# jby1993/SelfReconCode

Hardware: AMD Instinct MI355X
Metric: train.py-equivalent iterations/sec (540x540, 2048 rays/frame x 3 frames per GPU; coarse stage at Adam lr 0.0001) (higher is better)
Workload: dtype f32

## Files before the change

### include/selfrecon_hip.h

```cpp
#ifndef SELFRECON_HIP_H_
#define SELFRECON_HIP_H_
#include <stdint.h>

#ifdef __cplusplus
extern "C" {
#endif

#define SR_OK 0
#define SR_EINVAL (-1)
#define SR_ELAUNCH (-2)
#define SR_ENOSPC (-3)

int sr_abi_version(void);
const char* sr_build_arch(void);
const char* sr_build_digest(void);

int sr_minv3x3_fwd_f32(const float* ms, float* invs, uint8_t* checks, int64_t n, void* stream);
int sr_minv3x3_fwd_f64(const double* ms, double* invs, uint8_t* checks, int64_t n, void* stream);
int sr_minv3x3_bwd_f32(const float* grads, const float* invs, float* outs, int64_t n, void* stream);
int sr_minv3x3_bwd_f64(const double* grads, const double* invs, double* outs, int64_t n, void* stream);

typedef struct {
  int64_t size[5];
  int64_t stride[5];
} sr_tensor5;

int sr_gridsample3d_fwd_f32(const float* input, sr_tensor5 in_d, const float* grid, sr_tensor5 grid_d,
                            float* output, sr_tensor5 out_d, void* stream);
int sr_gridsample3d_fwd_f64(const double* input, sr_tensor5 in_d, const double* grid, sr_tensor5 grid_d,
                            double* output, sr_tensor5 out_d, void* stream);
int sr_gridsample3d_bwd_f32(const float* input, sr_tensor5 in_d, const float* grid, sr_tensor5 grid_d,
                            const float* grad_output, sr_tensor5 gout_d,
                            float* grad_input , sr_tensor5 gin_d, float* grad_grid, void* stream);
int sr_gridsample3d_bwd_f64(const double* input, sr_tensor5 in_d, const double* grid, sr_tensor5 grid_d,
                            const double* grad_output, sr_tensor5 gout_d,
                            double* grad_input , sr_tensor5 gin_d, double* grad_grid, void* stream);
int sr_gridsample3d_fwd_f16(const void* input, sr_tensor5 in_d, const void* grid, sr_tensor5 grid_d, void* output, sr_tensor5 out_d,
                            void* stream);
int sr_gridsample3d_bwd_f16(const void* input, sr_tensor5 in_d, const void* grid, sr_tensor5 grid_d, const void* grad_output,
                            sr_tensor5 gout_d, void* grad_input , sr_tensor5 gin_d, void* grad_grid, void* stream);
int sr_gridsample3d_dbwd_f16(const void* gO_input , sr_tensor5 goi_d, const void* gO_grid, sr_tensor5 gog_d,
                             const void* input, sr_tensor5 in_d, const void* grid, sr_tensor5 grid_d, const void* grad_output,
                             sr_tensor5 gout_d, void* grad_input , sr_tensor5 gin_d, void* grad_grid,
                             void* grad_grad_output, void* stream);
int sr_gridsample3d_dbwd_f32(const float* gO_input , sr_tensor5 goi_d, const float* gO_grid, sr_tensor5 gog_d,
                             const float* input, sr_tensor5 in_d, const float* grid, sr_tensor5 grid_d,
                             const float* grad_output, sr_tensor5 gout_d,
                             float* grad_input , sr_tensor5 gin_d, float* grad_grid, float* grad_grad_output,
                             void* stream);
int sr_gridsample3d_dbwd_f64(const double* gO_input , sr_tensor5 goi_d, const double* gO_grid, sr_tensor5 gog_d,
                             const double* input, sr_tensor5 in_d, const double* grid, sr_tensor5 grid_d,
                             const double* grad_output, sr_tensor5 gout_d,
                             double* grad_input , sr_tensor5 gin_d, double* grad_grid, double* grad_grad_output,
                             void* stream);


#define SR_ACT_NONE 0
#define SR_ACT_SOFTPLUS100 1
#define SR_ACT_RELU 2
#define SR_EPI_FWD 0
#define SR_EPI_BWD 1
typedef struct {
  const float* A; int64_t lda;
  const float* B; int64_t ldb;
  float* C; int64_t ldc;
  int32_t M, N, K;
  const float* bias;
  int32_t group, act, mode;
  float out_scale;
  const float* aux; int64_t ldaux;
  int32_t naux_fwd;
  int32_t nact_bwd;
  float aux_scale;
} sr_gemm_args;
int sr_mlp_gemm_nt(const sr_gemm_args* host_args, void* stream);
int sr_mlp_gemm_nt_tile(int32_t M, int32_t ncols, int32_t* bm_out, int32_t* bn_out);

#define SR_CHAIN_MAX_LAYERS 10
typedef struct {
  int32_t nlayers;
  int32_t nprob[SR_CHAIN_MAX_LAYERS];
  sr_gemm_args g[SR_CHAIN_MAX_LAYERS][2];
  const int32_t* m_dev; int32_t m_mul;
  int32_t m_cap;
} sr_chain_args;
int sr_mlp_chain(const sr_chain_args* host_args, void* stream);

typedef struct {
  const float* Z; int64_t ldz;
  const float* A; int64_t lda;
  float* dW; int64_t lddw;
  float* partial;
  int32_t R, N, K, splits, accumulate;
  float* db; float* db_partial; int32_t group;
} sr_gemm_tn_args;
int64_t sr_mlp_gemm_tn_workspace_floats(int32_t R, int32_t N, int64_t lddw, int32_t* host_splits_out);
int sr_mlp_gemm_tn(const sr_gemm_tn_args* host_args, void* stream);
#define SR_TN_GROUP_MAX 12
typedef struct {
  int32_t n;
  sr_gemm_tn_args p[SR_TN_GROUP_MAX];
} sr_gemm_tn_group_args;
int sr_mlp_gemm_tn_group(const sr_gemm_tn_group_args* host_args, void* stream);

int sr_pe_embed(const float* x, int64_t P, int32_t L, const float* band_weights, const float* extra, int64_t ldextra,
                int32_t E, const int64_t* extra_index , int32_t group, float* out, int64_t ldo, void* stream);
int sr_pe_embed_bwd(const float* x, int64_t P, int32_t L, const float* band_weights, int32_t group, const float* gA0,
                    int64_t ldg, float* xbar, void* stream);

typedef struct {
  const float* p; const float* tp; int64_t P;
  const float* A; const float* trans; int32_t nframes;
  const int64_t* batch_inds; int64_t points_per_frame;
  const float* vol; int32_t D, H, W;
  float bmin[3], bmax[3];
  float* y;
  float* jac;
} sr_lbs_args;
int sr_lbs_fwd(const sr_lbs_args* host_args, void* stream);
int64_t sr_lbs_bwd_workspace_floats(int64_t P, int32_t nframes);
int sr_lbs_bwd(const sr_lbs_args* host_args, const float* ybar, float* pbar, float* Abar, float* transbar, float* partials, void* stream);
int sr_lbs_jac_bwd(const sr_lbs_args* host_args, const float* ybar, const float* Jbar, float* pbar, float* Abar, float* transbar, float* partials,
                   void* stream);

int sr_lbs_chain_fwd(const float* poses, int32_t B, const float* host_Js, const int32_t* host_parents, const float* host_init_pose,
                     float* G, float* A, void* stream);
int sr_lbs_chain_bwd(const float* poses, int32_t B, const float* host_Js, const int32_t* host_parents, const float* host_init_pose,
                     const float* Abar, const float* Gbar, float* posebar, void* stream);

typedef struct {
  int64_t M; int32_t group;
  const float* sdf4; int64_t ld_sdf;
  const float* off4; int64_t ld_off;
  const float* y; const float* jlbs;
  const float* rays; const float* cam;
  const float* p; float* p_out;
  uint8_t* converged;
  float dthreshold, athreshold, w1, w2;
} sr_newton_args;
int sr_newton_update(const sr_newton_args* host_args, void* stream);

typedef struct {
  int64_t M;
  const float* sdf; int64_t ld_sdf;
  const float* y; const float* jlbs;
  const float* rays; const float* cam;
  uint8_t* converged;
  float* t_out; int64_t ld_t; float* s_out;
  const float* grad_f; const float* grad_off;
  const float* p; float* p_out;
  float dthreshold, athreshold, w1, w2;
} sr_newton2_args;
int sr_newton_prepare(const sr_newton2_args* host_args, void* stream);
int sr_newton_apply(const sr_newton2_args* host_args, void* stream);

typedef struct {
  int32_t P, times;
  const float* p0; const float* rays; const int64_t* batch_inds;
  const float* cam;
  int32_t L_sdf; const float* w_sdf; int32_t L_def; const float* w_def;
  const float* conds; int64_t ld_conds; int32_t E;
  const float* A; const float* trans; int32_t nframes;
  const float* vol; int32_t D, H, W; float bmin[3], bmax[3];
  float dthreshold, athreshold, w1, w2;
  int32_t* live;
  float* x[2]; float* v[2]; int32_t* frame[2]; int32_t* orig[2];
  float* unit;
  float* a0; int64_t ld_a0; float* a0d; int64_t ld_a0d;
  const float* sdf_out; int64_t ld_sdf; const float* def_out; int64_t ld_def;
  uint8_t* conv; float* t; float* s;
  const float* a0bar; int64_t ld_a0bar; const float* skipbar; int64_t ld_skipbar; int32_t n_skip;
  const float* a0dbar; int64_t ld_a0dbar;
  float* p_out; uint8_t* conv_out;
} sr_refine_args;
int sr_refine_init(const sr_refine_args* host_args, void* stream);
int sr_refine_embed(const sr_refine_args* host_args, int32_t phase, void* stream);
int sr_refine_mid(const sr_refine_args* host_args, int32_t phase, int32_t mode, void* stream);
int sr_refine_finish(const sr_refine_args* host_args, int32_t phase, void* stream);


int64_t sr_mc_workspace_bytes(int32_t nx, int32_t ny, int32_t nz);
int sr_mc_count(const float* sdf, int32_t nx, int32_t ny, int32_t nz, float iso, void* workspace, uint32_t* counts_dev, void* stream);
int sr_mc_emit(const float* sdf, int32_t nx, int32_t ny, int32_t nz, float iso, const void* workspace, float xstep, float ystep,
               float zstep, float xmin, float ymin, float zmin, float* verts, int64_t* faces, void* stream);

int sr_svd3x3(const float* A, int64_t n, float* U, float* S, float* V, void* stream);

int sr_rows_pad(const float* a, int64_t lda, int32_t na, const float* b, int64_t ldb, int32_t nb, int64_t rows, int32_t group, float* dst, int64_t ldd,
                int32_t width, void* stream);
int64_t sr_rows_frame_sum_workspace_floats(int64_t P, int32_t E, int32_t n);
int sr_rows_frame_sum(const float* X, int64_t ldx, int64_t P, int32_t E, const int64_t* index, int32_t n, float* partial, float* out, void* stream);

#define SR_PACK_MAX_LAYERS 16
typedef struct { const float* v; const float* g; float* W; float* WT; float* norms; int32_t N, K; int64_t ldw, ldwt; } sr_pack_layer;
typedef struct { int32_t nlayers; sr_pack_layer layer[SR_PACK_MAX_LAYERS]; } sr_pack_table;
typedef struct { const float* dW; int64_t lddw; const float* v; const float* g; const float* norms; float* gv; float* gg;
                 const float* db; float* gb;
                 int32_t N, K, accumulate, pad_; } sr_unpack_layer;
typedef struct { int32_t nlayers; sr_unpack_layer layer[SR_PACK_MAX_LAYERS]; } sr_unpack_table;
int sr_pack_weights(const sr_pack_table* host_table, void* stream);
int sr_unpack_grads(const sr_unpack_table* host_table, void* stream);

#define SR_ADAM_MAX_TENSORS 64
typedef struct { float* p; const float* g; float* m; float* v; int64_t numel; float lr, bias1, inv_sqrt_bias2, pad_; } sr_adam_tensor;
typedef struct { int32_t ntensors; float beta1, beta2, eps;
                 float one_minus_beta1, one_minus_beta2;
                 int32_t pad_[2]; sr_adam_tensor tensor[SR_ADAM_MAX_TENSORS]; } sr_adam_table;
int sr_adam_step(const sr_adam_table* host_table, void* stream);

int sr_stream_stamp(uint64_t* out, void* stream);
int sr_stream_flag_set(uint32_t* flag, uint32_t value, void* stream);
int sr_stream_flag_wait(const uint32_t* flag, uint32_t value, uint32_t* timed_out, int32_t timeout_ms, void* stream);

int sr_interp2x3d_fwd_f32(const float* in, int64_t BC, int32_t d, int32_t h, int32_t w, float balance, float* out, uint8_t* is_boundary, void* stream);
int sr_interp2x3d_fwd_f64(const double* in, int64_t BC, int32_t d, int32_t h, int32_t w, float balance, double* out, uint8_t* is_boundary, void* stream);
int sr_interp2x3d_bwd_f32(const float* grad_out, int64_t BC, int32_t d, int32_t h, int32_t w, float* grad_in, void* stream);
int sr_interp2x3d_bwd_f64(const double* grad_out, int64_t BC, int32_t d, int32_t h, int32_t w, double* grad_in, void* stream);
int sr_seg3d_candidates(const uint8_t* is_boundary, const uint8_t* done, int32_t D, int32_t H, int32_t W, int64_t* out_index, uint64_t* count_dev,
                        void* stream);

int64_t sr_points_silhouette_workspace_bytes(int64_t nimg, int64_t pts_per_img, int32_t H, int32_t W, float radius);
int sr_points_silhouette_fwd(const float* xy_ndc, const float* z, int64_t nimg, int64_t pts_per_img, int32_t H, int32_t W, float radius,
                             int32_t K, float* mask, void* workspace, void* stream);
int sr_points_silhouette_bwd(const float* xy_ndc, const float* z, int64_t nimg, int64_t pts_per_img, int32_t H, int32_t W, float radius,
                             const void* workspace, const float* gmask, float* gxy, void* stream);
int sr_rasterize_meshes(const float* xy_ndc, const float* z, const int64_t* faces, int64_t nimg, int64_t V, int64_t F, int32_t H, int32_t W,
                        void* zbuf_u64, int64_t* pix_to_face, float* bary, float* zout, void* stream);

int sr_vertex_adjacency(const int64_t* faces, int64_t V, int64_t F, int64_t* offsets, int32_t* cursor, int32_t* nbr, void* stream);
int sr_vertex_normals(const float* verts, int64_t N, int64_t V, const int64_t* offsets, const int32_t* nbr, float* normals, void* stream);
int sr_shade_phong(const float* verts, const float* normals, const int64_t* faces, int64_t N, int64_t V, int64_t F, int32_t H, int32_t W,
                   const int64_t* pix_to_face, const float* bary, const float* cam_pos, const float* light_loc, const float* host_phong,
                   float* rgba, void* stream);

#define SR_STEP_MAX_FRAMES 8
typedef struct { const float* R; const float* T; const float* f; const float* c; float W, H, one_minus_inv_w, one_minus_inv_h; } sr_camera;
int sr_step_reduce_blocks(int64_t rows);
int sr_step_param_blocks(int64_t rows);
int sr_cam_project_ndc_fwd(const float* ps, int64_t n, const sr_camera* cam, float* xy, float* z, void* stream);
int sr_cam_project_ndc_bwd(const float* ps, int64_t n, const sr_camera* cam, const float* gxy, const float* gz, float* gps, float* partial,
                           float* gparams, void* stream);
int sr_cam_view_rays_fwd(const float* pixels, int64_t n, const sr_camera* cam, float* rays, void* stream);
int sr_cam_view_rays_bwd(const float* pixels, int64_t n, const sr_camera* cam, const float* grays, float* partial, float* gparams, void* stream);

int sr_cardinal_rays_fwd(const float* J, const float* v, int64_t n, float* out, uint8_t* ok, void* stream);
int sr_cardinal_rays_bwd(const float* J, const float* v, int64_t n, const float* gout, float* gJ, float* gv, void* stream);
int sr_deformed_normals(const float* J, const float* onx, int64_t n, float* out, void* stream);

#define SR_STEP_LOSS_SLOTS (1 + 2 * SR_STEP_MAX_FRAMES)
typedef struct { const int64_t* b; const int64_t* r; const int64_t* c; int64_t P; int32_t N, H, W; } sr_ray_pixels;
int sr_color_loss_fwd(const sr_ray_pixels* px, const float* colors, const float* gt, float* partial, float* out, void* stream);
int sr_color_loss_bwd(const sr_ray_pixels* px, const float* colors, const float* gt, const float* saved, const float* gloss, float* gcolors,
                      void* stream);
int sr_normal_loss_fwd(const sr_ray_pixels* px, const float* nx_raw, const float* J, const float* gt_normals, const float* R, const float* rays,
                       int weighted, float* partial, float* out, void* stream);
int sr_normal_loss_bwd(const sr_ray_pixels* px, const float* nx_raw, const float* J, const float* gt_normals, const float* R, const float* rays,
                       int weighted, const float* saved, const float* gloss, float* gnx_raw, float* gJ, void* stream);
int sr_eikonal_loss_fwd(const float* g, int64_t n, float* partial, float* out, void* stream);
int sr_eikonal_loss_bwd(const float* g, int64_t n, const float* gloss, float* gg, void* stream);
int sr_def_regu_loss_fwd(const float* S, int64_t n, float c, float* partial, float* out, void* stream);
int sr_def_regu_loss_bwd(const float* U, const float* S, const float* V, int64_t n, float c, const float* gloss, float* gJ, void* stream);
int sr_svd3x3_bwd(const float* U, const float* V, const float* gS, int64_t n, float* gJ, void* stream);
int sr_mask_iou_loss_fwd(const float* masks, const float* gt, int N, int64_t hw, float* partial, float* out, void* stream);
int sr_mask_iou_loss_bwd(const float* masks, const float* gt, int N, int64_t hw, const float* saved, const float* gloss, float* gmasks, void* stream);

int sr_implicit_solve(const float* grad_f, const float* J, const float* v, const float* grad_l, int64_t n, float* cot_f, float* rhs_tail, float* temp,
                      uint8_t* ok, void* stream);

int sr_uv_rasterize(const float* vt, const int64_t* ft, int64_t Vt, int64_t F, int32_t R, int32_t* face, float* bary, void* stream);
int sr_face_visibility(const int64_t* pix_to_face, const int64_t* faces, int64_t N, int64_t V, int64_t F, const float* xy_pix, const uint8_t* mask,
                       int32_t H, int32_t W, uint8_t* visible, void* stream);
int sr_view_alpha(const float* verts, const float* normals, const float* cam_pos, int64_t N, int64_t V, float* alpha, void* stream);
int sr_texture_accumulate(int64_t T, const int32_t* tface, const float* tbary, const int64_t* faces, int64_t F, int64_t V, int32_t N,
                          const uint8_t* visible, const float* alpha, const float* xy_pix, const float* images, int32_t H, int32_t W,
                          const int32_t* fids, int32_t agg_num, float cosv0, float* slot_cos, float* slot_rgb, int32_t* slot_view, int32_t* count,
                          float* min_cos, int32_t* min_idx, void* stream);
int sr_texture_resolve(int64_t T, const int32_t* texel, int32_t agg_num, float cosv0, int32_t check_num, const float* slot_cos,
                       const float* slot_rgb, const int32_t* slot_view, int32_t* count, uint8_t* mask_final, int32_t* view_id, float* tex_median,
                       void* stream);
int64_t sr_texture_fill_workspace_bytes(int32_t R);
int sr_texture_fill(const float* tex_median, const uint8_t* mask_final, const uint8_t* tex_mask, int32_t R, int32_t dilate, float* texture,
                    void* workspace, void* stream);

#define SR_QUADRIC_CLAMPED 1
#define SR_QUADRIC_NO_PLANES 2
int sr_meshprep_cell_faces(const int64_t* faces, int64_t F, const int64_t* vertex_map, int64_t V, int64_t C, int64_t* slot, void* stream);
int sr_meshprep_cell_quadric(const float* verts, int64_t V, const int64_t* faces, int64_t F, const int64_t* face_slots, const int64_t* face_offsets,
                             const int64_t* order, const int64_t* offsets, const int64_t* cells, int64_t C, const float* lo, float cell, int64_t nx,
                             int64_t ny, double reg, float* out, int32_t* flags, float* shift, void* stream);
int sr_meshprep_face_flips(const float* verts, int64_t V, const int64_t* faces, int64_t F, const float* new_verts, int64_t Vn,
                           const int64_t* new_faces, const int64_t* source, int64_t Fn, int64_t* counts, void* stream);
int sr_meshprep_bounds(const float* verts, int64_t V, int32_t* box, void* stream);
int sr_meshprep_cell_keys(const float* verts, int64_t V, const float* lo, float cell, int64_t nx, int64_t ny, int64_t nz, int64_t* key, void* stream);
int sr_meshprep_cell_mean(const float* verts, int64_t V, const int64_t* order, const int64_t* offsets, int64_t C, float* out, void* stream);
int sr_meshprep_face_keys(const int64_t* faces, int64_t F, const int64_t* vertex_map, int64_t V, int64_t Vn, int64_t* out_faces, int64_t* key_hi,
                          int64_t* key_lo, void* stream);
int sr_meshprep_face_first(const int64_t* key_hi, const int64_t* key_lo, const int64_t* perm, int64_t F, uint8_t* keep, void* stream);
int sr_chart_classify(const float* verts, int64_t V, const int64_t* faces, int64_t F, int32_t* cls, void* stream);
int sr_chart_edge_keys(const int64_t* faces, int64_t F, int64_t V, const int32_t* cls, int64_t* key, void* stream);
int sr_chart_hook(const int64_t* sorted_key, const int64_t* perm, int64_t n, const int32_t* parent, int32_t* next, int64_t F, int32_t* changed,
                  void* stream);
int sr_chart_jump(const int32_t* parent, int64_t F, int32_t* next, int32_t* changed, void* stream);
int sr_chart_bbox(const float* verts, int64_t V, const int64_t* faces, int64_t F, const int32_t* cls, const int64_t* chart, int64_t C, int32_t* box,
                  float* bbox_min, float* extent, void* stream);
int sr_chart_uv(const float* verts, int64_t V, const int64_t* faces, int64_t F, const int32_t* cls, const int64_t* chart, int64_t C,
                const float* bbox_min, const int64_t* origin, double scale, int32_t padding, int32_t R, float* vt, void* stream);
int sr_uv_overlap_count(const float* vt, const int64_t* ft, int64_t Vt, int64_t F, int32_t R, double eps, int32_t* count, int64_t* total,
                        void* stream);

int sr_collapse_vertex_quadrics(const float* verts, int64_t V, const int64_t* faces, int64_t F, const int64_t* slots, const int64_t* offsets,
                                double* quadrics, void* stream);
int sr_collapse_edge_keys(const int64_t* faces, int64_t F, int64_t V, int64_t* key, void* stream);
int sr_collapse_edge_heads(const int64_t* unique_key, const int64_t* offsets, int64_t E, const int64_t* perm, const int64_t* faces, int64_t F, int64_t V,
                           int64_t* edges, int32_t* count, int64_t* opposite, int32_t* locked, int64_t* directed, void* stream);
int sr_collapse_candidates(const float* verts, int64_t V, const int64_t* faces, int64_t F, const double* quadrics, const int64_t* slots,
                           const int64_t* offsets, const int64_t* neighbours, const int64_t* neighbour_offsets, const int64_t* edges,
                           const int32_t* count, const int64_t* opposite, const int32_t* locked, int64_t E, double reg, double flip_cos,
                           float* positions, int64_t* key, void* stream);
int sr_collapse_min1(const int64_t* edges, const int64_t* key, int64_t E, int64_t V, int64_t* m1, void* stream);
int sr_collapse_min2(const int64_t* edges, int64_t E, int64_t V, const int64_t* m1, int64_t* m2, void* stream);
int sr_collapse_select(const int64_t* edges, const int64_t* key, int64_t E, int64_t V, const int64_t* m2, uint8_t* selected, int64_t* record,
                       void* stream);
int sr_collapse_apply_vertices(const int64_t* edges, const float* positions, const uint8_t* selected, int64_t E, float* verts, int64_t V,
                               double* quadrics, int64_t* target, void* stream);
int sr_collapse_apply_faces(const int64_t* faces, int64_t F, const int64_t* target, int64_t V, int64_t* out_faces, uint8_t* keep, void* stream);
int sr_collapse_map_jump(const int64_t* parent, int64_t V, int64_t* next, int32_t* changed, void* stream);

int sr_texture_mips(const void* texture, int32_t is_u8, const uint8_t* valid, int32_t R, float* mips, void* stream);
int sr_texture_face_lod(const float* xy_pix, const int64_t* faces, const float* vt, const int64_t* ft, int64_t N, int64_t V, int64_t F,
                        int64_t Vt, int32_t R, float bias, int32_t L, float* lod, void* stream);
int sr_shade_textured(const int64_t* pix_to_face, const float* bary, int64_t N, int64_t F, int32_t H, int32_t W, const int64_t* ft,
                      const float* vt, int64_t Vt, const float* mips, int32_t R, int32_t L, const float* lod, const float* host_background,
                      const float* host_hole, const float* bg_image, float* rgba, float* coverage, void* stream);

#define SR_LBSW_MAX_K 32
int sr_lbsw_knn_blend(const float* verts, const float* vert_ws, int64_t nv, int32_t nj, int32_t k, int32_t W, int32_t H, int32_t D,
                      const float* bmin, const float* bmax, int32_t align_corners, float* field, void* stream);
int sr_lbsw_smooth(const float* src, float* dst, int32_t nj, int32_t W, int32_t H, int32_t D, void* stream);

#define SR_SMPL_BATCH_TILE 8
int sr_smpl_shape(const float* v_template, const float* shapedirs, const float* beta, int32_t B, int32_t nbeta, int64_t nv, float* v_shaped,
                  void* stream);
int64_t sr_smpl_regress_workspace_floats(int32_t B, int64_t nv, int32_t nk);
int sr_smpl_regress(const float* x, const float* reg, int32_t B, int64_t nv, int32_t nk, float* partial, float* out, void* stream);
int sr_smpl_pose(const float* theta, float* Rs, const float* J, const int32_t* host_parents, int32_t B, float* feature, float* J_transformed,
                 float* A, void* stream);
int sr_smpl_skin(const float* rest, int64_t rest_batch_stride, const float* posedirs, const float* feature, const float* weights, const float* A,
                 int32_t B, int64_t nv, float* verts, void* stream);

int sr_smpl_regress_bwd(const float* g_out, const float* reg, int32_t B, int64_t nv, int32_t nk, int32_t accumulate, float* g_x, void* stream);
int64_t sr_smpl_shape_bwd_workspace_floats(int32_t B, int32_t nbeta, int64_t nv);
int sr_smpl_shape_bwd(const float* shapedirs, const float* g_vshaped, int32_t B, int32_t nbeta, int64_t nv, float* partial, float* g_beta,
                      void* stream);
int64_t sr_smpl_skin_bwd_workspace_floats(int32_t B, int64_t nv);
int sr_smpl_skin_bwd(const float* rest, int64_t rest_batch_stride, const float* posedirs, const float* feature, const float* weights,
                     const float* A, const float* gV, int32_t B, int64_t nv, float* partial, float* g_rest, float* gA, float* g_feature,
                     void* stream);
int sr_smpl_pose_bwd(const float* theta, const float* Rs, const float* J, const float* A, const int32_t* host_parents, int32_t B,
                     const float* gA, const float* gJ_transformed, const float* g_feature, const float* gRs, float* g_theta, float* gRs_out,
                     float* gJ, void* stream);

int sr_keypoint_energy(const float* joints, const float* trans, const float* kp, const float* joint_weights, const float* host_camera,
                       float sigma, int32_t T, int32_t K, float* energy, float* g_joints, float* g_trans, int32_t* behind, void* stream);

#define SR_EDT_EMPTY 1073741824
int sr_edt(const uint8_t* mask, int32_t F, int32_t H, int32_t W, int32_t* d2, void* stream);
int sr_contour_flags(const uint8_t* mask, int32_t F, int32_t H, int32_t W, uint8_t* flags, void* stream);
int sr_silhouette_energy(const float* points, const int32_t* d2, const int32_t* samples, const int32_t* counts, const float* host_camera,
                         float sigma, float margin, int32_t F, int32_t V, int32_t S, int32_t H, int32_t W, float* xy, uint8_t* valid,
                         float* vres, int32_t* match, float* sres, float* e_in, float* e_cov, int32_t* outside, float* g_points, void* stream);

#define SR_MESHREG_LAP 1
#define SR_MESHREG_EDGE 2
#define SR_MESHREG_NORMAL 4
int64_t sr_meshreg_workspace_bytes(int64_t V, int64_t P);
int sr_meshreg_fwd(const float* verts, int64_t V, const int32_t* nbr_row, const int32_t* nbr, int64_t E, const int32_t* pairs, int64_t P,
                   int32_t terms, float target_length, float* lap_q, float* edge_g, float* pair_g, void* workspace, float* out, void* stream);
int sr_meshreg_bwd(int64_t V, const int32_t* nbr_row, const int32_t* nbr, int64_t E, const int32_t* pair_row, const int32_t* pair_ent, int64_t P,
                   const float* lap_q, const float* edge_g, const float* pair_g, const float* g_lap, const float* g_edge, const float* g_nc,
                   float* grad, void* stream);

#define SR_FRAMES_MAX_BATCH 16
#define SR_FRAMES_MAX_PIXELS 1073741824
struct sr_frame_ids_s {
  int32_t id[SR_FRAMES_MAX_BATCH];
};
typedef struct sr_frame_ids_s sr_frame_ids;
int sr_frames_fetch(const uint8_t* img_u8, const uint8_t* normal_u8, const uint8_t* mask_u8, int64_t pitch3, int64_t pitch1, int32_t F, int32_t H,
                    int32_t W, const sr_frame_ids* ids_by_value, const int64_t* ids_device, int32_t N, float* out_img, float* out_normal,
                    float* out_mask, void* stream);

#define SR_LOG_MAX_SLOTS 32
#define SR_LOG_EMPTY 0
#define SR_LOG_F32 1
#define SR_LOG_I64 2
#define SR_LOG_IMM 3
struct sr_log_slots_s {
  const void* src[SR_LOG_MAX_SLOTS];
  float imm[SR_LOG_MAX_SLOTS];
  uint8_t kind[SR_LOG_MAX_SLOTS];
};
typedef struct sr_log_slots_s sr_log_slots;
int sr_log_row(const sr_log_slots* slots_by_value, int32_t n, float* ring, int32_t ring_rows, int32_t ld, int64_t row, void* stream);

#define SR_JPEG_BLOCK_BYTES 208
int sr_jpeg_transform(const uint8_t* rgb, int32_t B, int32_t H, int32_t W, const uint16_t* qtab, int16_t* coef, void* stream);
int sr_jpeg_entropy(const int16_t* coef, int32_t B, int32_t H, int32_t W, const uint32_t* huff, uint32_t* bits, int64_t bits_dwords,
                    uint8_t* rowbuf, int64_t rowbuf_bytes, uint32_t* row_len, void* stream);
int sr_jpeg_gather(const uint8_t* rowbuf, const uint32_t* row_len, int32_t B, int32_t H, int32_t W, int64_t* row_start, uint8_t* out,
                   int64_t out_bytes, int64_t* offsets, void* stream);

int sr_surfdist_face_cells(const float* tri, int64_t F, const float* lo, float cell, int32_t nx, int32_t ny, int32_t nz, int64_t* count, void* stream);
int sr_surfdist_emit_pairs(const float* tri, int64_t F, const float* lo, float cell, int32_t nx, int32_t ny, int32_t nz, const int64_t* offset,
                           int64_t pairs, int64_t* key, int32_t* pair_face, void* stream);
int sr_surfdist_query(const float* points, int64_t P, const float* tri, int64_t F, const float* lo, float cell, int32_t nx, int32_t ny, int32_t nz,
                      const int64_t* cell_start, const int32_t* cell_faces, int64_t pairs, float* dist, int64_t* face, float* closest, void* stream);
int sr_surfdist_brute(const float* points, int64_t P, const float* tri, int64_t F, float* dist, int64_t* face, float* closest, void* stream);
int sr_mesh_sample(const float* tri, const double* cum_area, int64_t F, int64_t n, int64_t seed, float* points, int64_t* face, float* normals,
                   void* stream);

#define SR_ICP_MAX_BLOCKS 1024
#define SR_ICP_COLS 40
#define SR_ICP_HISTORY 6
#define SR_ICP_STATE 16
#define SR_ICP_DONE 12
int sr_icp_accumulate(const float* points, int64_t S, const float* tri, int64_t F, const float* lo, float cell, int32_t nx, int32_t ny, int32_t nz,
                      const int64_t* cell_start, const int32_t* cell_faces, int64_t pairs, const double* state, double ox, double oy, double oz,
                      double rho, float max_dist, int32_t measure, double* partial, int32_t blocks, void* stream);
int sr_icp_solve(const double* partial, int32_t blocks, double ox, double oy, double oz, double rho, int32_t scale, double tol, int32_t it,
                 int32_t iters, double* state, double* history, void* stream);
int sr_icp_score(const float* points, int64_t S, const double* table, int32_t N, const float* tri, int64_t F, const float* lo, float cell,
                 int32_t nx, int32_t ny, int32_t nz, const int64_t* cell_start, const int32_t* cell_faces, int64_t pairs, const float* trunc,
                 double* score, void* stream);

#ifdef __cplusplus
}
#endif
#endif
```

### selfreconcode_amd/csrc/mlp_gemm.hip

```cpp
#include "sr_common.h"
#include <stdlib.h>
#include <type_traits>

typedef float f32x16 __attribute__((ext_vector_type(16)));
typedef float f32x4 __attribute__((ext_vector_type(4)));
typedef int i32x4 __attribute__((ext_vector_type(4)));

__device__ __forceinline__ __amdgpu_buffer_rsrc_t sr_make_rsrc(const void* base, int64_t bytes) {
  return __builtin_amdgcn_make_buffer_rsrc(const_cast<void*>(base), 0, (int)(bytes < 0xFFFFFFFFll ? bytes : 0xFFFFFFFFll), 0x00020000);
}
__device__ __forceinline__ f32x4 sr_buffer_load16(__amdgpu_buffer_rsrc_t rsrc, uint32_t lane_off, uint32_t scalar_off) {
  return __builtin_bit_cast(f32x4, __builtin_amdgcn_raw_buffer_load_b128(rsrc, (int)lane_off, (int)scalar_off, 0));
}

namespace {

constexpr int BK = 32;
constexpr int LDSP = BK + 4;

__device__ __forceinline__ float fast_exp(float x) { return __builtin_amdgcn_exp2f(x * 1.4426950408889634f); }
__device__ __forceinline__ float fast_log(float x) { return __builtin_amdgcn_logf(x) * 0.6931471805599453f; }
__device__ __forceinline__ float softplus100(float z) {
  const float t = z * 100.0f;
  const float e = fast_exp(fminf(t, 20.0f));
  const float l = e < 1e-3f ? e * (1.0f - e * (0.5f - e * 0.33333334f)) : fast_log(1.0f + e);
  return t > 20.0f ? z : l * 0.01f;
}
__device__ __forceinline__ float dsoftplus100(float z) {
  const float t = z * 100.0f;
  const float e = fast_exp(fminf(t, 20.0f));
  return t > 20.0f ? 1.0f : e * __builtin_amdgcn_rcpf(e + 1.0f);
}
__device__ __forceinline__ void softplus100_from_stored(float x, float& d, float& c2) {
  const float em = fast_exp(-x);
  d = x < 1e-3f ? x * (1.0f - x * (0.5f - x * 0.16666667f)) : 1.0f - em;
  c2 = 100.0f * em;
}

template <int WM, int WN, int TM, int TN>
struct Cfg {
  static constexpr int kWaves = WM * WN;
  static constexpr int kThreads = kWaves * 64;
  static constexpr int BM = WM * TM * 32;
  static constexpr int BN = WN * TN * 32;
  static constexpr int kALoads = BM * (BK / 4) / kThreads;
  static constexpr int kBLoads = (BN * (BK / 4) + kThreads - 1) / kThreads;
  static constexpr int kOperandFloats = 2 * (BM + BN) * LDSP;
  static constexpr int kStageFloats = kWaves * TM * 32 * (TN * 32 + 4);
  static constexpr int kLdsFloats = kOperandFloats > kStageFloats ? kOperandFloats : kStageFloats;
};

template <int ROWS, int NLOADS, int THREADS>
struct TileLoader {
  const float* p[NLOADS];
  __amdgpu_buffer_rsrc_t rsrc;
  uint32_t off[NLOADS];
  int kq4;
  int K, kmax;
  __device__ __forceinline__ TileLoader(const float* __restrict__ P, int64_t ld, int R, int K_, int r0) : K(K_) {
    kq4 = (threadIdx.x & 7) * 4;
    kmax = ((K_ + 3) & ~3) - 4;
    const int rb = r0 < R ? r0 : R - 1;
    rsrc = sr_make_rsrc(P + (int64_t)rb * ld, (int64_t)(R - rb) * ld * 4);
#pragma unroll
    for (int j = 0; j < NLOADS; ++j) {
      int row = (threadIdx.x + j * THREADS) >> 3;
      if (row >= ROWS) row = ROWS - 1;
      int gr = r0 + row;
      if (gr >= R) gr = R - 1;
      p[j] = P + (int64_t)gr * ld;
      off[j] = (uint32_t)(((int64_t)(gr - rb) * ld + kq4) * 4);
    }
  }
  __device__ __forceinline__ void load(int k0, f32x4 (&reg)[NLOADS]) const {
    const int gk = k0 + kq4;
    const int gkc = gk < kmax ? gk : kmax;
#pragma unroll
    for (int j = 0; j < NLOADS; ++j) reg[j] = *reinterpret_cast<const f32x4*>(p[j] + gkc);
  }
  __device__ __forceinline__ void load_full(int k0, int klast, f32x4 (&reg)[NLOADS]) const {
    const uint32_t kc = (uint32_t)(k0 < klast ? k0 : klast) * 4u;
#pragma unroll
    for (int j = 0; j < NLOADS; ++j) reg[j] = sr_buffer_load16(rsrc, off[j], kc);
  }
  template <bool KTAIL = true>
  __device__ __forceinline__ void store(float* __restrict__ lds, int k0, const f32x4 (&reg)[NLOADS]) const {
    const int nvalid = K - (k0 + kq4);
#pragma unroll
    for (int j = 0; j < NLOADS; ++j) {
      const int idx = threadIdx.x + j * THREADS;
      const int row = idx >> 3;
      f32x4 v = reg[j];
      if (KTAIL) { v.x = nvalid > 0 ? v.x : 0.f; v.y = nvalid > 1 ? v.y : 0.f; v.z = nvalid > 2 ? v.z : 0.f; v.w = nvalid > 3 ? v.w : 0.f; }
      if (ROWS * 8 % THREADS == 0 || row < ROWS) *reinterpret_cast<f32x4*>(lds + row * LDSP + kq4) = v;
    }
  }
};

template <int WM, int WN, int TM, int TN, int G>
__device__ __forceinline__ void epilogue(const sr_gemm_args& g, f32x16 (&acc)[TM][TN], int m0, int n0, int wm, int wn,
                                         int li, int kh, float* __restrict__ stage) {
  constexpr int SP = TN * 32 + 4;
  const int ncols = g.N + g.naux_fwd;
  const float inv_aux_scale = 1.0f / g.aux_scale;
#pragma unroll
  for (int a = 0; a < TM; ++a) {
#pragma unroll
    for (int b = 0; b < TN; ++b) {
      const int col = n0 + (wn * TN + b) * 32 + li;
      if (col >= ncols) continue;
      const float bias = (g.bias && col < g.N) ? g.bias[col] : 0.f;
#pragma unroll
      for (int q = 0; q < 4; ++q) {
        const int r0 = m0 + (wm * TM + a) * 32 + 8 * q + 4 * kh;
        if (r0 >= g.M) continue;
        float v[4] = {acc[a][b][4 * q], acc[a][b][4 * q + 1], acc[a][b][4 * q + 2], acc[a][b][4 * q + 3]};
        float o[4];
        if (g.mode == SR_EPI_FWD) {
          if (col >= g.N) {
#pragma unroll
            for (int j = 0; j < 4; ++j) o[j] = (r0 + j < g.M) ? g.aux[(int64_t)(r0 + j) * g.ldaux + (col - g.N)] * g.out_scale : 0.f;
          } else {
#pragma unroll
            for (int s = 0; s < 4; s += G) {
              const float z = v[s] + bias;
              float d;
              if (g.act == SR_ACT_SOFTPLUS100) { o[s] = softplus100(z) * g.out_scale; d = (G > 1) ? dsoftplus100(z) : 0.f; }
              else if (g.act == SR_ACT_RELU) { o[s] = fmaxf(z, 0.f) * g.out_scale; d = z > 0.f ? 1.f : 0.f; }
              else { o[s] = z * g.out_scale; d = 1.f; }
#pragma unroll
              for (int tI = 1; tI < G; ++tI) o[s + tI] = d * v[s + tI] * g.out_scale;
            }
          }
        } else {
          if (col >= g.nact_bwd) {
#pragma unroll
            for (int j = 0; j < 4; ++j) o[j] = v[j] * g.out_scale;
          } else {
            float sv[4];
#pragma unroll
            for (int j = 0; j < 4; ++j) sv[j] = (r0 + j < g.M) ? g.aux[(int64_t)(r0 + j) * g.ldaux + col] : 0.f;
#pragma unroll
            for (int s = 0; s < 4; s += G) {
              float d, c2;
              if (g.act == SR_ACT_SOFTPLUS100) {
                softplus100_from_stored(100.0f * (sv[s] * inv_aux_scale), d, c2);
              } else if (g.act == SR_ACT_RELU) { d = sv[s] > 0.f ? 1.f : 0.f; c2 = 0.f; }
              else { d = 1.f; c2 = 0.f; }
              float cross = 0.f;
#pragma unroll
              for (int tI = 1; tI < G; ++tI) {
                cross += sv[s + tI] * v[s + tI];
                o[s + tI] = d * g.aux_scale * v[s + tI];
              }
              o[s] = d * g.aux_scale * v[s] + c2 * cross;
            }
          }
        }
        float* sp = stage + (a * 32 + 8 * q + 4 * kh) * SP + b * 32 + li;
#pragma unroll
        for (int j = 0; j < 4; ++j) sp[j * SP] = o[j];
      }
    }
  }
  __syncthreads();
  constexpr int QPR = TN * 8;
  constexpr int RPI = 64 / QPR;
  const int lane = kh * 32 + li;
  const int qc = lane % QPR, ro = lane / QPR;
  const int col0 = n0 + wn * TN * 32 + qc * 4;
#pragma unroll
  for (int i = 0; i < TM * 32 / RPI; ++i) {
    const int lr = i * RPI + ro;
    const int row = m0 + wm * TM * 32 + lr;
    if (row >= g.M || col0 >= ncols) continue;
    const f32x4 v = *reinterpret_cast<const f32x4*>(stage + lr * SP + qc * 4);
    float* dst = g.C + (int64_t)row * g.ldc + col0;
    if (col0 + 3 < ncols) {
      *reinterpret_cast<f32x4*>(dst) = v;
    } else {
      dst[0] = v.x;
      if (col0 + 1 < ncols) dst[1] = v.y;
      if (col0 + 2 < ncols) dst[2] = v.z;
    }
  }
}

template <int WM, int WN, int TM, int TN, int G, int MODE, int ACT>
__device__ __forceinline__ void epilogue_interior(const sr_gemm_args& g, f32x16 (&acc)[TM][TN], int m0, int n0, int wm, int wn, int li,
                                                  int kh, float* __restrict__ stage) {
  constexpr int SP = TN * 32 + 4;
  const float os = g.out_scale, as = g.aux_scale, inv_as = 1.0f / g.aux_scale;
#pragma unroll
  for (int a = 0; a < TM; ++a) {
#pragma unroll
    for (int b = 0; b < TN; ++b) {
      const int col = n0 + (wn * TN + b) * 32 + li;
      const float bias = (MODE == SR_EPI_FWD && g.bias) ? g.bias[col] : 0.f;
#pragma unroll
      for (int q = 0; q < 4; ++q) {
        const int r0 = m0 + (wm * TM + a) * 32 + 8 * q + 4 * kh;
        const float v[4] = {acc[a][b][4 * q], acc[a][b][4 * q + 1], acc[a][b][4 * q + 2], acc[a][b][4 * q + 3]};
        float o[4];
        if constexpr (MODE == SR_EPI_FWD) {
#pragma unroll
          for (int s = 0; s < 4; s += G) {
            const float z = v[s] + bias;
            float d = 1.f;
            if constexpr (ACT == SR_ACT_SOFTPLUS100) { o[s] = softplus100(z) * os; if (G > 1) d = dsoftplus100(z); }
            else if constexpr (ACT == SR_ACT_RELU) { o[s] = fmaxf(z, 0.f) * os; d = z > 0.f ? 1.f : 0.f; }
            else { o[s] = z * os; }
#pragma unroll
            for (int tI = 1; tI < G; ++tI) o[s + tI] = d * v[s + tI] * os;
          }
        } else {
          float sv[4];
          if constexpr (ACT != SR_ACT_NONE || G > 1) {
            const float* ap = g.aux + (int64_t)r0 * g.ldaux + col;
#pragma unroll
            for (int j = 0; j < 4; ++j) sv[j] = ap[(int64_t)j * g.ldaux];
          }
#pragma unroll
          for (int s = 0; s < 4; s += G) {
            float d = 1.f, c2 = 0.f;
            if constexpr (ACT == SR_ACT_SOFTPLUS100) softplus100_from_stored(100.0f * (sv[s] * inv_as), d, c2);
            else if constexpr (ACT == SR_ACT_RELU) d = sv[s] > 0.f ? 1.f : 0.f;
            float cross = 0.f;
#pragma unroll
            for (int tI = 1; tI < G; ++tI) {
              cross += sv[s + tI] * v[s + tI];
              o[s + tI] = d * as * v[s + tI];
            }
            o[s] = d * as * v[s] + c2 * cross;
          }
        }
        float* sp = stage + (a * 32 + 8 * q + 4 * kh) * SP + b * 32 + li;
#pragma unroll
        for (int j = 0; j < 4; ++j) sp[j * SP] = o[j];
      }
    }
  }
  __syncthreads();
  constexpr int QPR = TN * 8, RPI = 64 / QPR;
  const int lane = kh * 32 + li;
  const int qc = lane % QPR, ro = lane / QPR;
  float* dst = g.C + (int64_t)(m0 + wm * TM * 32 + ro) * g.ldc + n0 + wn * TN * 32 + qc * 4;
#pragma unroll
  for (int i = 0; i < TM * 32 / RPI; ++i)
    *reinterpret_cast<f32x4*>(dst + (int64_t)i * RPI * g.ldc) = *reinterpret_cast<const f32x4*>(stage + (i * RPI + ro) * SP + qc * 4);
}

template <int WM, int WN, int TM, int TN, int G, int MODE>
__device__ __forceinline__ void epilogue_interior_act(const sr_gemm_args& g, f32x16 (&acc)[TM][TN], int m0, int n0, int wm, int wn, int li,
                                                      int kh, float* __restrict__ stage) {
  if (g.act == SR_ACT_SOFTPLUS100) epilogue_interior<WM, WN, TM, TN, G, MODE, SR_ACT_SOFTPLUS100>(g, acc, m0, n0, wm, wn, li, kh, stage);
  else if (g.act == SR_ACT_RELU) epilogue_interior<WM, WN, TM, TN, G, MODE, SR_ACT_RELU>(g, acc, m0, n0, wm, wn, li, kh, stage);
  else epilogue_interior<WM, WN, TM, TN, G, MODE, SR_ACT_NONE>(g, acc, m0, n0, wm, wn, li, kh, stage);
}

struct NoProbe { __device__ __forceinline__ void operator()(int) const {} };
template <int WM, int WN, int TM, int TN, bool KTAIL = true, class Probe = NoProbe>
__device__ __forceinline__ void gemm_nt_tile(const sr_gemm_args& g, int wg, float* __restrict__ smem, Probe probe = Probe()) {
  using C_ = Cfg<WM, WN, TM, TN>;
  auto As = [&](int buf) -> float* { return smem + buf * (C_::BM * LDSP); };
  auto Bs = [&](int buf) -> float* { return smem + 2 * C_::BM * LDSP + buf * (C_::BN * LDSP); };

  const int tiles_n = (g.N + g.naux_fwd + C_::BN - 1) / C_::BN;
  const int tiles_m = (g.M + C_::BM - 1) / C_::BM;
  const int nwg = tiles_m * tiles_n;
  {
    const int q = nwg / 8, r = nwg % 8, xcd = wg % 8, loc = wg / 8;
    wg = (xcd < r ? xcd * (q + 1) : r * (q + 1) + (xcd - r) * q) + loc;
  }
  const int tn = wg % tiles_n, tm = wg / tiles_n;
  const int m0 = tm * C_::BM, n0 = tn * C_::BN;

  const int lane = threadIdx.x & 63, wave = threadIdx.x >> 6;
  const int wm = wave / WN, wn = wave % WN;
  const int li = lane & 31, kh = lane >> 5;

  f32x16 acc[TM][TN];
#pragma unroll
  for (int a = 0; a < TM; ++a)
#pragma unroll
    for (int b = 0; b < TN; ++b)
#pragma unroll
      for (int r = 0; r < 16; ++r) acc[a][b][r] = 0.f;

  const TileLoader<C_::BM, C_::kALoads, C_::kThreads> la(g.A, g.lda, g.M, g.K, m0);
  const TileLoader<C_::BN, C_::kBLoads, C_::kThreads> lb(g.B, g.ldb, g.N, g.K, n0);
  const int nk = (g.K + BK - 1) / BK;
  const int a_off = (wm * TM * 32 + li) * LDSP + kh * 4, b_off = (wn * TN * 32 + li) * LDSP + kh * 4;
  f32x4 fa0[2][TM], fb0[2][TN], fa1[2][TM], fb1[2][TN];
  auto read_frags = [&](const float* abuf, const float* bbuf, int kk0, f32x4 (&fa)[2][TM], f32x4 (&fb)[2][TN]) {
#pragma unroll
    for (int h = 0; h < 2; ++h) {
#pragma unroll
      for (int a = 0; a < TM; ++a) fa[h][a] = *reinterpret_cast<const f32x4*>(abuf + a_off + a * 32 * LDSP + (kk0 + h) * 8);
#pragma unroll
      for (int b = 0; b < TN; ++b) fb[h][b] = *reinterpret_cast<const f32x4*>(bbuf + b_off + b * 32 * LDSP + (kk0 + h) * 8);
    }
  };
  auto mfma_kk = [&](const f32x4 (&fa)[TM], const f32x4 (&fb)[TN]) {
#pragma unroll
    for (int e = 0; e < 4; ++e)
#pragma unroll
      for (int a = 0; a < TM; ++a)
#pragma unroll
        for (int b = 0; b < TN; ++b) acc[a][b] = __builtin_amdgcn_mfma_f32_32x32x2f32(fa[a][e], fb[b][e], acc[a][b], 0, 0, 0);
  };
  constexpr int kMem = C_::kALoads + C_::kBLoads;

  f32x4 ra0[C_::kALoads], rb0[C_::kBLoads], ra1[C_::kALoads], rb1[C_::kBLoads];
  const int klast = (nk - 1) * BK;
  auto load_tile = [&](int k0, f32x4 (&ar)[C_::kALoads], f32x4 (&br)[C_::kBLoads]) {
    if constexpr (KTAIL) { la.load(k0, ar); lb.load(k0, br); }
    else { la.load_full(k0, klast, ar); lb.load_full(k0, klast, br); }
  };
  load_tile(0, ra0, rb0);
  load_tile(BK, ra1, rb1);
  la.template store<KTAIL>(As(0), 0, ra0); lb.template store<KTAIL>(Bs(0), 0, rb0);
  __syncthreads();
  read_frags(As(0), Bs(0), 0, fa0, fb0);
  probe(0);
  auto step = [&](int t, f32x4 (&ain)[C_::kALoads], f32x4 (&bin)[C_::kBLoads], const f32x4 (&aout)[C_::kALoads],
                  const f32x4 (&bout)[C_::kBLoads]) {
    const int cur = t & 1;
    load_tile((t + 2) * BK, ain, bin);
    la.template store<KTAIL>(As(cur ^ 1), (t + 1) * BK, aout); lb.template store<KTAIL>(Bs(cur ^ 1), (t + 1) * BK, bout);
    read_frags(As(cur), Bs(cur), 2, fa1, fb1);
    mfma_kk(fa0[0], fb0[0]);
    mfma_kk(fa0[1], fb0[1]);
#pragma unroll
    for (int i = 0; i < kMem; ++i) {
      __builtin_amdgcn_sched_group_barrier(0x020, 1, 0);
      __builtin_amdgcn_sched_group_barrier(0x008, 1, 0);
    }
#pragma unroll
    for (int i = 0; i < kMem; ++i) {
      __builtin_amdgcn_sched_group_barrier(0x200, 1, 0);
      __builtin_amdgcn_sched_group_barrier(0x008, 1, 0);
    }
#pragma unroll
    for (int i = 0; i < 2 * (TM + TN); ++i) {
      __builtin_amdgcn_sched_group_barrier(0x100, 1, 0);
      __builtin_amdgcn_sched_group_barrier(0x008, 1, 0);
    }
    __builtin_amdgcn_sched_barrier(0);
    __syncthreads();
    read_frags(As(cur ^ 1), Bs(cur ^ 1), 0, fa0, fb0);
    __builtin_amdgcn_sched_barrier(0);
    mfma_kk(fa1[0], fb1[0]);
    mfma_kk(fa1[1], fb1[1]);
    __builtin_amdgcn_sched_barrier(0);
  };
  for (int t = 0; t < nk; t += 2) {
    step(t, ra0, rb0, ra1, rb1);
    if (t + 1 < nk) step(t + 1, ra1, rb1, ra0, rb0);
  }
  __syncthreads();
  probe(1);

  float* stage = smem + wave * (TM * 32 * (TN * 32 + 4));
  const bool interior = m0 + C_::BM <= g.M && n0 + C_::BN <= (g.mode == SR_EPI_FWD ? g.N : (g.nact_bwd < g.N ? g.nact_bwd : g.N));
  if (interior) {
    if (g.mode == SR_EPI_FWD) {
      switch (g.group) {
        case 1: epilogue_interior_act<WM, WN, TM, TN, 1, SR_EPI_FWD>(g, acc, m0, n0, wm, wn, li, kh, stage); break;
        case 2: epilogue_interior_act<WM, WN, TM, TN, 2, SR_EPI_FWD>(g, acc, m0, n0, wm, wn, li, kh, stage); break;
        default: epilogue_interior_act<WM, WN, TM, TN, 4, SR_EPI_FWD>(g, acc, m0, n0, wm, wn, li, kh, stage); break;
      }
    } else {
      switch (g.group) {
        case 1: epilogue_interior_act<WM, WN, TM, TN, 1, SR_EPI_BWD>(g, acc, m0, n0, wm, wn, li, kh, stage); break;
        case 2: epilogue_interior_act<WM, WN, TM, TN, 2, SR_EPI_BWD>(g, acc, m0, n0, wm, wn, li, kh, stage); break;
        default: epilogue_interior_act<WM, WN, TM, TN, 4, SR_EPI_BWD>(g, acc, m0, n0, wm, wn, li, kh, stage); break;
      }
    }
  } else {
    switch (g.group) {
      case 1: epilogue<WM, WN, TM, TN, 1>(g, acc, m0, n0, wm, wn, li, kh, stage); break;
      case 2: epilogue<WM, WN, TM, TN, 2>(g, acc, m0, n0, wm, wn, li, kh, stage); break;
      default: epilogue<WM, WN, TM, TN, 4>(g, acc, m0, n0, wm, wn, li, kh, stage); break;
    }
  }
  probe(2);
}

template <int WM, int WN, int TM, int TN, bool KTAIL>
__global__ __launch_bounds__(WM * WN * 64) __attribute__((amdgpu_waves_per_eu(2))) void gemm_nt_kernel(sr_gemm_args g) {
  extern __shared__ __attribute__((aligned(16))) float smem[];
  gemm_nt_tile<WM, WN, TM, TN, KTAIL>(g, blockIdx.x, smem);
}


using ChainCfg = Cfg<2, 2, 1, 1>;

constexpr int TBR = 32;
template <int ZW, int XW>
struct TnCfg {
  static constexpr int ZLD = ZW + 4, XLD = XW + 4;
  static constexpr int kZ = TBR * ZLD, kX = TBR * XLD;
  static constexpr int kLdsFloats = 2 * (kZ + kX);
  static constexpr int TLZ = TBR * (ZW / 4) / 256, TLX = TBR * (XW / 4) / 256;
  static constexpr int WN = XW / 64;
};

template <int ZW, int XW>
__device__ __forceinline__ void gemm_tn_body(const sr_gemm_tn_args& g, int rows_per_split, int bid, int nblocks, float* __restrict__ tn_smem) {
  using C = TnCfg<ZW, XW>;
  auto Zs = [&](int buf) -> float* { return tn_smem + buf * C::kZ; };
  auto Xs = [&](int buf) -> float* { return tn_smem + 2 * C::kZ + buf * C::kX; };
  const int tiles_k = (g.K + XW - 1) / XW;
  const int tiles_n = (g.N + ZW - 1) / ZW;
  int vb = bid;
  if ((nblocks & 7) == 0) vb = (bid & 7) * (nblocks >> 3) + (bid >> 3);
  const int tile = vb % (tiles_k * tiles_n), split = vb / (tiles_k * tiles_n);
  const int n0 = (tile / tiles_k) * ZW, k0 = (tile % tiles_k) * XW;
  const int r_begin = split * rows_per_split;
  const int r_end = min(g.R, r_begin + rows_per_split);
  const int lane = threadIdx.x & 63, wave = threadIdx.x >> 6;
  const int wm = wave / C::WN, wn = wave % C::WN, li = lane & 31, kh = lane >> 5;

  f32x16 acc[2][2];
#pragma unroll
  for (int a = 0; a < 2; ++a)
#pragma unroll
    for (int b = 0; b < 2; ++b)
#pragma unroll
      for (int r = 0; r < 16; ++r) acc[a][b][r] = 0.f;

  constexpr int TLZ = C::TLZ, TLX = C::TLX;
  constexpr int ZT = ZW / 4, XT = XW / 4;
  const int cqz = (threadIdx.x % ZT) * 4, lrz = threadIdx.x / ZT;
  const int cqx = (threadIdx.x % XT) * 4, lrx = threadIdx.x / XT;
  const int zmax = ((g.N + 3) & ~3) - 4, xmax = ((g.K + 3) & ~3) - 4;
  const float* zcol = g.Z + (n0 + cqz < zmax ? n0 + cqz : zmax);
  const float* xcol = g.A + (k0 + cqx < xmax ? k0 + cqx : xmax);
  f32x4 rz[TLZ], rx[TLX];
  const __amdgpu_buffer_rsrc_t zrsrc = sr_make_rsrc(g.Z + (int64_t)r_begin * g.ldz, (int64_t)(g.R - r_begin) * g.ldz * 4);
  const __amdgpu_buffer_rsrc_t xrsrc = sr_make_rsrc(g.A + (int64_t)r_begin * g.lda, (int64_t)(g.R - r_begin) * g.lda * 4);
  uint32_t zbyte[TLZ], xbyte[TLX];
#pragma unroll
  for (int j = 0; j < TLZ; ++j) zbyte[j] = (uint32_t)(((int64_t)(lrz + j * (256 / ZT)) * g.ldz + (zcol - g.Z)) * 4);
#pragma unroll
  for (int j = 0; j < TLX; ++j) xbyte[j] = (uint32_t)(((int64_t)(lrx + j * (256 / XT)) * g.lda + (xcol - g.A)) * 4);
  const int last_full = r_end - TBR;
  auto load = [&](int r0, auto tail) {
    if constexpr (decltype(tail)::value) {
#pragma unroll
      for (int j = 0; j < TLZ; ++j) {
        int gr = r0 + lrz + j * (256 / ZT);
        gr = gr < r_end ? gr : r_end - 1;
        rz[j] = *reinterpret_cast<const f32x4*>(zcol + (int64_t)gr * g.ldz);
      }
#pragma unroll
      for (int j = 0; j < TLX; ++j) {
        int gr = r0 + lrx + j * (256 / XT);
        gr = gr < r_end ? gr : r_end - 1;
        rx[j] = *reinterpret_cast<const f32x4*>(xcol + (int64_t)gr * g.lda);
      }
    } else {
      const int rc = r0 < last_full ? r0 : last_full;
      const uint32_t zo = (uint32_t)((int64_t)(rc - r_begin) * g.ldz * 4), xo = (uint32_t)((int64_t)(rc - r_begin) * g.lda * 4);
#pragma unroll
      for (int j = 0; j < TLZ; ++j) rz[j] = sr_buffer_load16(zrsrc, zbyte[j], zo);
#pragma unroll
      for (int j = 0; j < TLX; ++j) rx[j] = sr_buffer_load16(xrsrc, xbyte[j], xo);
    }
  };
  auto store = [&](int buf, int r0, auto tail) {
    float* zs = Zs(buf);
    float* xs = Xs(buf);
#pragma unroll
    for (int j = 0; j < TLZ; ++j) {
      const int row = lrz + j * (256 / ZT);
      f32x4 z = rz[j];
      if constexpr (decltype(tail)::value) {
        const bool ok = r0 + row < r_end;
        z.x = ok ? z.x : 0.f; z.y = ok ? z.y : 0.f; z.z = ok ? z.z : 0.f; z.w = ok ? z.w : 0.f;
      }
      *reinterpret_cast<f32x4*>(zs + row * C::ZLD + cqz) = z;
    }
#pragma unroll
    for (int j = 0; j < TLX; ++j) {
      const int row = lrx + j * (256 / XT);
      f32x4 x = rx[j];
      if constexpr (decltype(tail)::value) {
        const bool ok = r0 + row < r_end;
        x.x = ok ? x.x : 0.f; x.y = ok ? x.y : 0.f; x.z = ok ? x.z : 0.f; x.w = ok ? x.w : 0.f;
      }
      *reinterpret_cast<f32x4*>(xs + row * C::XLD + cqx) = x;
    }
  };

  constexpr int HS = TBR / 4;
  typedef float f32x2 __attribute__((ext_vector_type(2)));
  float z0a[HS], z1a[HS], x0a[HS], x1a[HS], z0b[HS], z1b[HS], x0b[HS], x1b[HS];
  const int zoff = kh * C::ZLD + wm * 64 + 2 * li, xoff = kh * C::XLD + wn * 64 + 2 * li;
  auto read_half = [&](int buf, int half, float (&z0)[HS], float (&z1)[HS], float (&x0)[HS], float (&x1)[HS]) {
    const float* zb = Zs(buf) + zoff + half * HS * 2 * C::ZLD;
    const float* xb = Xs(buf) + xoff + half * HS * 2 * C::XLD;
#pragma unroll
    for (int e = 0; e < HS; ++e) {
      const f32x2 z = *reinterpret_cast<const f32x2*>(zb + 2 * e * C::ZLD), x = *reinterpret_cast<const f32x2*>(xb + 2 * e * C::XLD);
      z0[e] = z.x; z1[e] = z.y; x0[e] = x.x; x1[e] = x.y;
    }
  };
  auto mfma_half = [&](const float (&z0)[HS], const float (&z1)[HS], const float (&x0)[HS], const float (&x1)[HS]) {
#pragma unroll
    for (int e = 0; e < HS; ++e) {
      acc[0][0] = __builtin_amdgcn_mfma_f32_32x32x2f32(z0[e], x0[e], acc[0][0], 0, 0, 0);
      acc[0][1] = __builtin_amdgcn_mfma_f32_32x32x2f32(z0[e], x1[e], acc[0][1], 0, 0, 0);
      acc[1][0] = __builtin_amdgcn_mfma_f32_32x32x2f32(z1[e], x0[e], acc[1][0], 0, 0, 0);
      acc[1][1] = __builtin_amdgcn_mfma_f32_32x32x2f32(z1[e], x1[e], acc[1][1], 0, 0, 0);
    }
  };

  const bool do_bias = g.db_partial != nullptr && k0 == 0;
  const float wodd = g.group == 4 ? 0.f : 1.f;
  float bsum0 = 0.f, bsum1 = 0.f;
  auto bias_half = [&](const float (&z0)[HS], const float (&z1)[HS]) {
#pragma unroll
    for (int e = 0; e < HS; ++e) {
      if (e & 1) { bsum0 += wodd * z0[e]; bsum1 += wodd * z1[e]; }
      else { bsum0 += z0[e]; bsum1 += z1[e]; }
    }
  };
  const int nsteps = (r_end - r_begin + TBR - 1) / TBR;
  auto run = [&](auto tail, auto bias) {
    load(r_begin, tail);
    store(0, r_begin, tail);
    load(r_begin + TBR, tail);
    __syncthreads();
    read_half(0, 0, z0a, z1a, x0a, x1a);
    for (int t = 0; t < nsteps; ++t) {
      const int cur = t & 1;
      store(cur ^ 1, r_begin + (t + 1) * TBR, tail);
      load(r_begin + (t + 2) * TBR, tail);
      read_half(cur, 1, z0b, z1b, x0b, x1b);
      mfma_half(z0a, z1a, x0a, x1a);
#pragma unroll
      for (int i = 0; i < TLZ + TLX; ++i) {
        __builtin_amdgcn_sched_group_barrier(0x200, 1, 0);
        __builtin_amdgcn_sched_group_barrier(0x008, 1, 0);
      }
#pragma unroll
      for (int i = 0; i < TLZ + TLX; ++i) {
        __builtin_amdgcn_sched_group_barrier(0x020, 1, 0);
        __builtin_amdgcn_sched_group_barrier(0x008, 1, 0);
      }
#pragma unroll
      for (int i = 0; i < HS; ++i) {
        __builtin_amdgcn_sched_group_barrier(0x100, 1, 0);
        __builtin_amdgcn_sched_group_barrier(0x008, 1, 0);
      }
      __builtin_amdgcn_sched_barrier(0);
      if constexpr (decltype(bias)::value) bias_half(z0a, z1a);
      __builtin_amdgcn_sched_barrier(0);
      __syncthreads();
      read_half(cur ^ 1, 0, z0a, z1a, x0a, x1a);
      __builtin_amdgcn_sched_barrier(0);
      mfma_half(z0b, z1b, x0b, x1b);
      if constexpr (decltype(bias)::value) bias_half(z0b, z1b);
      __builtin_amdgcn_sched_barrier(0);
    }
  };
  if (nsteps > 0) {
    const bool tail = ((r_end - r_begin) % TBR) != 0;
    if (tail) {
      if (do_bias) run(std::true_type{}, std::true_type{}); else run(std::true_type{}, std::false_type{});
    } else {
      if (do_bias) run(std::false_type{}, std::true_type{}); else run(std::false_type{}, std::false_type{});
    }
  }
  __syncthreads();
  if (do_bias) {
    float* red = Zs(0);
    if (wn == 0) {
      const bool use = kh == 0 || g.group == 1;
      red[kh * ZW + wm * 64 + 2 * li] = use ? bsum0 : 0.f;
      red[kh * ZW + wm * 64 + 2 * li + 1] = use ? bsum1 : 0.f;
    }
    __syncthreads();
    if (threadIdx.x < ZW && n0 + threadIdx.x < g.N) g.db_partial[(int64_t)split * g.N + n0 + threadIdx.x] = red[threadIdx.x] + red[threadIdx.x + ZW];
  }
  float* out = g.partial + (int64_t)split * g.N * g.lddw;
#pragma unroll
  for (int a = 0; a < 2; ++a)
#pragma unroll
    for (int b = 0; b < 2; ++b) {
      const int col = k0 + wn * 64 + 2 * li + b;
      if (col >= g.K) continue;
#pragma unroll
      for (int r = 0; r < 16; ++r) {
        const int row = n0 + wm * 64 + 2 * ((r & 3) + 8 * (r >> 2) + 4 * kh) + a;
        if (row < g.N) out[(int64_t)row * g.lddw + col] = acc[a][b][r];
      }
    }
}

template <int ZW, int XW>
__global__ __launch_bounds__(256) __attribute__((amdgpu_waves_per_eu(2))) void gemm_tn_kernel(sr_gemm_tn_args g, int rows_per_split) {
  extern __shared__ __attribute__((aligned(16))) float tn_smem[];
  gemm_tn_body<ZW, XW>(g, rows_per_split, blockIdx.x, gridDim.x, tn_smem);
}

struct TnGroup {
  int n;
  int first[SR_TN_GROUP_MAX + 1];
  int blocks[SR_TN_GROUP_MAX];
  int rows_per_split[SR_TN_GROUP_MAX];
  sr_gemm_tn_args p[SR_TN_GROUP_MAX];
};
__global__ __launch_bounds__(256) __attribute__((amdgpu_waves_per_eu(2))) void gemm_tn_group_kernel(TnGroup G) {
  extern __shared__ __attribute__((aligned(16))) float tn_smem[];
  int i = 0;
  while (i + 1 < G.n && (int)blockIdx.x >= G.first[i + 1]) ++i;
  const int bid = blockIdx.x - G.first[i];
  if (bid >= G.blocks[i]) return;
  gemm_tn_body<128, 128>(G.p[i], G.rows_per_split[i], bid, G.blocks[i], tn_smem);
}

static inline bool tn_narrow(int N, int64_t K) { return K <= 64 && N >= 256; }

__device__ __forceinline__ void slab_reduce_body(const float* __restrict__ partial, float* __restrict__ dW, int N,
                                                 int K, int64_t lddw, int splits, int accumulate,
                                                 const float* __restrict__ db_partial, float* __restrict__ db, int bid, int nblocks) {
  const int64_t total = (int64_t)N * lddw;
  const int64_t quads = total >> 2;
  const int64_t all = quads + (db ? N : 0);
  const f32x4* __restrict__ p4 = reinterpret_cast<const f32x4*>(partial);
  f32x4* __restrict__ d4 = reinterpret_cast<f32x4*>(dW);
  for (int64_t i = (int64_t)bid * blockDim.x + threadIdx.x; i < all; i += (int64_t)nblocks * blockDim.x) {
    if (i < quads) {
      const int col = (int)((i << 2) % lddw);
      f32x4 s = {0.f, 0.f, 0.f, 0.f};
      if (col < K) {
        const f32x4* src = p4 + i;
        int p = 0;
        for (; p + 8 <= splits; p += 8) {
          f32x4 v[8];
#pragma unroll
          for (int j = 0; j < 8; ++j) v[j] = src[(int64_t)(p + j) * quads];
#pragma unroll
          for (int j = 0; j < 8; ++j) s += v[j];
        }
        for (; p < splits; ++p) s += src[(int64_t)p * quads];
        if (col + 1 >= K) s.y = 0.f;
        if (col + 2 >= K) s.z = 0.f;
        if (col + 3 >= K) s.w = 0.f;
      }
      f32x4 o = {0.f, 0.f, 0.f, 0.f};
      if (accumulate) o = d4[i];
      d4[i] = o + s;
    } else {
      const int n = (int)(i - quads);
      float s = 0.f;
      for (int p = 0; p < splits; ++p) s += db_partial[(int64_t)p * N + n];
      db[n] = (accumulate ? db[n] : 0.f) + s;
    }
  }
}

__global__ __launch_bounds__(256) void slab_reduce_kernel(const float* __restrict__ partial, float* __restrict__ dW, int N,
                                                           int K, int64_t lddw, int splits, int accumulate,
                                                           const float* __restrict__ db_partial, float* __restrict__ db) {
  slab_reduce_body(partial, dW, N, K, lddw, splits, accumulate, db_partial, db, blockIdx.x, gridDim.x);
}

__global__ __launch_bounds__(256) void slab_reduce_group_kernel(TnGroup G) {
  int i = 0;
  while (i + 1 < G.n && (int)blockIdx.x >= G.first[i + 1]) ++i;
  const int bid = blockIdx.x - G.first[i];
  if (bid >= G.blocks[i]) return;
  const sr_gemm_tn_args& g = G.p[i];
  slab_reduce_body(g.partial, g.dW, g.N, g.K, g.lddw, g.R > 0 ? g.splits : 0, g.accumulate, g.db_partial, g.db, bid, G.blocks[i]);
}

}

static void nt_tile_choice(int M, int ncols, int* bm, int* bn) {
  auto cost = [&](int tm, int tn, double eff) {
    const int64_t wgs = sr_cdiv(M, tm) * sr_cdiv(ncols, tn);
    return (double)sr_cdiv(wgs, 256) * tm * tn / eff;
  };
  if (ncols <= 32) {
    const double c[3] = {cost(32, 32, 0.6), cost(64, 32, 0.8), cost(256, 32, 1.0)};
    *bn = 32;
    if (c[0] < c[1] && c[0] < c[2]) *bm = 32;
    else if (c[1] < c[2]) *bm = 64;
    else *bm = 256;
  } else {
    const double c[3] = {cost(64, 64, 0.92), cost(64, 128, 0.94), cost(128, 128, 1.0)};
    int pick = 1;
    for (int i = 1; i < 3; ++i) if (c[i] < c[pick - 1]) pick = i + 1;
    *bm = pick == 3 ? 128 : 64;
    *bn = pick == 1 ? 64 : 128;
  }
}

extern "C" {
int sr_mlp_gemm_nt(const sr_gemm_args* a, void* stream) {
  if (!a || a->M < 0 || a->N <= 0 || a->K <= 0) return SR_EINVAL;
  if (a->M == 0) return SR_OK;
  if (!a->A || !a->B || !a->C) return SR_EINVAL;
  if (a->group != 1 && a->group != 2 && a->group != 4) return SR_EINVAL;
  if ((a->lda & 3) || (a->ldb & 3) || (a->ldc & 3) || ((uintptr_t)a->A & 15) || ((uintptr_t)a->B & 15) || ((uintptr_t)a->C & 15)) return SR_EINVAL;
  if (a->mode != SR_EPI_FWD && a->mode != SR_EPI_BWD) return SR_EINVAL;
  if ((a->naux_fwd > 0 || a->mode == SR_EPI_BWD) && a->act != SR_ACT_NONE && !a->aux && a->mode == SR_EPI_BWD) return SR_EINVAL;
  if (a->mode == SR_EPI_FWD && a->naux_fwd > 0 && !a->aux) return SR_EINVAL;
  if (a->M == 0) return SR_OK;
  if (a->M % a->group) return SR_EINVAL;
  const int ncols = a->N + (a->mode == SR_EPI_FWD ? a->naux_fwd : 0);
  sr_gemm_args g = *a;
  if (g.mode != SR_EPI_FWD) g.naux_fwd = 0;
#define SR_NT_LAUNCH(WM, WN, TM, TN)                                                                                        \
  do {                                                                                                                      \
    using C_ = Cfg<WM, WN, TM, TN>;                                                                                         \
    const int nwg = (int)(sr_cdiv(g.M, C_::BM) * sr_cdiv(ncols, C_::BN));                                                   \
    if (g.K % BK)                                                                                                           \
      hipLaunchKernelGGL((gemm_nt_kernel<WM, WN, TM, TN, true>), dim3(nwg), dim3(C_::kThreads), C_::kLdsFloats * sizeof(float), \
                         (hipStream_t)stream, g);                                                                           \
    else                                                                                                                    \
      hipLaunchKernelGGL((gemm_nt_kernel<WM, WN, TM, TN, false>), dim3(nwg), dim3(C_::kThreads), C_::kLdsFloats * sizeof(float), \
                         (hipStream_t)stream, g);                                                                           \
  } while (0)
  int bm = 0, bn = 0;
  nt_tile_choice(g.M, ncols, &bm, &bn);
  switch (bm * 1024 + bn) {
    case 32 * 1024 + 32: SR_NT_LAUNCH(1, 1, 1, 1); break;
    case 64 * 1024 + 32: SR_NT_LAUNCH(2, 1, 1, 1); break;
    case 256 * 1024 + 32: SR_NT_LAUNCH(4, 1, 2, 1); break;
    case 64 * 1024 + 64: SR_NT_LAUNCH(2, 2, 1, 1); break;
    case 64 * 1024 + 128: SR_NT_LAUNCH(2, 2, 1, 2); break;
    default: SR_NT_LAUNCH(2, 2, 2, 2); break;
  }
#undef SR_NT_LAUNCH
  return sr_launch_status();
}

int sr_mlp_gemm_nt_tile(int32_t M, int32_t ncols, int32_t* bm, int32_t* bn) {
  if (M <= 0 || ncols <= 0 || !bm || !bn) return SR_EINVAL;
  nt_tile_choice(M, ncols, bm, bn);
  return SR_OK;
}

__global__ __launch_bounds__(ChainCfg::kThreads) __attribute__((amdgpu_waves_per_eu(2))) void mlp_layer_pair_kernel(sr_gemm_args g0, sr_gemm_args g1, int nprob,
                                                                                                                     const int32_t* __restrict__ m_dev, int m_mul) {
  extern __shared__ __attribute__((aligned(16))) float smem[];
  const int M = *m_dev * m_mul;
  if (M <= 0) return;
  const int rows = (M + ChainCfg::BM - 1) / ChainCfg::BM;
  const int t0 = rows * ((g0.N + (g0.mode == SR_EPI_FWD ? g0.naux_fwd : 0) + ChainCfg::BN - 1) / ChainCfg::BN);
  const int t1 = nprob > 1 ? rows * ((g1.N + (g1.mode == SR_EPI_FWD ? g1.naux_fwd : 0) + ChainCfg::BN - 1) / ChainCfg::BN) : 0;
  const int t = blockIdx.x;
  if (t >= t0 + t1) return;
  if (t < t0) { g0.M = M; if (g0.K % BK) gemm_nt_tile<2, 2, 1, 1, true>(g0, t, smem); else gemm_nt_tile<2, 2, 1, 1, false>(g0, t, smem); }
  else { g1.M = M; if (g1.K % BK) gemm_nt_tile<2, 2, 1, 1, true>(g1, t - t0, smem); else gemm_nt_tile<2, 2, 1, 1, false>(g1, t - t0, smem); }
}

int sr_mlp_chain(const sr_chain_args* a, void* stream) {
  if (!a || a->nlayers < 1 || a->nlayers > SR_CHAIN_MAX_LAYERS || !a->m_dev || a->m_mul < 1 || a->m_cap <= 0) return SR_EINVAL;
  for (int l = 0; l < a->nlayers; ++l) {
    if (a->nprob[l] < 1 || a->nprob[l] > 2) return SR_EINVAL;
    for (int p = 0; p < a->nprob[l]; ++p) {
      const sr_gemm_args& g = a->g[l][p];
      if (!g.A || !g.B || !g.C || g.N <= 0 || g.K <= 0 || g.group != a->m_mul) return SR_EINVAL;
      if ((g.lda & 3) || (g.ldb & 3) || (g.ldc & 3) || ((uintptr_t)g.A & 15) || ((uintptr_t)g.B & 15) || ((uintptr_t)g.C & 15)) return SR_EINVAL;
      if (g.mode != SR_EPI_FWD && g.mode != SR_EPI_BWD) return SR_EINVAL;
      if (g.mode == SR_EPI_BWD && g.naux_fwd != 0) return SR_EINVAL;
      if ((g.mode == SR_EPI_BWD && g.act != SR_ACT_NONE && !g.aux) || (g.mode == SR_EPI_FWD && g.naux_fwd > 0 && !g.aux)) return SR_EINVAL;
    }
  }
  const int64_t rows = sr_cdiv((int64_t)a->m_cap * a->m_mul, ChainCfg::BM);
  for (int l = 0; l < a->nlayers; ++l) {
    int64_t tiles = 0;
    for (int p = 0; p < a->nprob[l]; ++p) {
      const sr_gemm_args& g = a->g[l][p];
      tiles += rows * sr_cdiv(g.N + (g.mode == SR_EPI_FWD ? g.naux_fwd : 0), ChainCfg::BN);
    }
    hipLaunchKernelGGL(mlp_layer_pair_kernel, dim3((unsigned)tiles), dim3(ChainCfg::kThreads), ChainCfg::kLdsFloats * sizeof(float), (hipStream_t)stream,
                       a->g[l][0], a->g[l][a->nprob[l] > 1 ? 1 : 0], a->nprob[l], a->m_dev, a->m_mul);
  }
  return sr_launch_status();
}

int64_t sr_mlp_gemm_tn_workspace_floats(int32_t R, int32_t N, int64_t lddw, int32_t* splits_out) {
  const int tiles = tn_narrow(N, lddw) ? (int)sr_cdiv(N, 256) : (int)(sr_cdiv(N, 128) * sr_cdiv(lddw, 128));
  const int target = 512;
  int splits = (int)sr_cdiv(target, tiles);
  const int max_splits = (int)sr_cdiv(R, 384);
  if (splits > max_splits) splits = max_splits;
  if (splits < 1) splits = 1;
  if (splits_out) *splits_out = splits;
  return (int64_t)splits * N * lddw;
}

int sr_mlp_gemm_tn(const sr_gemm_tn_args* a, void* stream) {
  if (!a || !a->dW || !a->partial || a->R < 0 || a->N <= 0 || a->K <= 0 || a->splits < 1) return SR_EINVAL;
  if (a->R > 0 && (!a->Z || !a->A)) return SR_EINVAL;
  if ((a->ldz & 3) || (a->lda & 3) || ((uintptr_t)a->Z & 15) || ((uintptr_t)a->A & 15) || a->lddw < a->K) return SR_EINVAL;
  if ((a->lddw & 3) || ((uintptr_t)a->dW & 15) || ((uintptr_t)a->partial & 15)) return SR_EINVAL;
  if ((a->db != nullptr) != (a->db_partial != nullptr) || (a->db && a->group < 1)) return SR_EINVAL;
  const bool narrow = tn_narrow(a->N, a->lddw);
  const int tiles = narrow ? (int)sr_cdiv(a->N, 256) : (int)(sr_cdiv(a->N, 128) * sr_cdiv(a->K, 128));
  int rows_per_split = (int)sr_cdiv(a->R, a->splits);
  rows_per_split = (int)(sr_cdiv(rows_per_split, TBR) * TBR);
  if (a->R > 0) {
    using Narrow = TnCfg<256, 64>;
    using Square = TnCfg<128, 128>;
    if (narrow)
      hipLaunchKernelGGL((gemm_tn_kernel<256, 64>), dim3(tiles * a->splits), dim3(256), Narrow::kLdsFloats * sizeof(float), (hipStream_t)stream, *a,
                         rows_per_split);
    else
      hipLaunchKernelGGL((gemm_tn_kernel<128, 128>), dim3(tiles * a->splits), dim3(256), Square::kLdsFloats * sizeof(float), (hipStream_t)stream, *a,
                         rows_per_split);
  }
  const int64_t total = (int64_t)a->N * a->lddw / 4 + (a->db ? a->N : 0);
  sr_launch_stream(slab_reduce_kernel, total, 256, stream, a->partial, a->dW, a->N, a->K, a->lddw, a->R > 0 ? a->splits : 0, a->accumulate, a->db_partial,
                   a->db);
  return sr_launch_status();
}

static int tn_check(const sr_gemm_tn_args* a) {
  if (!a || !a->dW || !a->partial || a->R < 0 || a->N <= 0 || a->K <= 0 || a->splits < 1) return SR_EINVAL;
  if (a->R > 0 && (!a->Z || !a->A)) return SR_EINVAL;
  if ((a->ldz & 3) || (a->lda & 3) || ((uintptr_t)a->Z & 15) || ((uintptr_t)a->A & 15) || a->lddw < a->K) return SR_EINVAL;
  if ((a->lddw & 3) || ((uintptr_t)a->dW & 15) || ((uintptr_t)a->partial & 15)) return SR_EINVAL;
  if ((a->db != nullptr) != (a->db_partial != nullptr) || (a->db && a->group < 1)) return SR_EINVAL;
  return SR_OK;
}

int sr_mlp_gemm_tn_group(const sr_gemm_tn_group_args* a, void* stream) {
  if (!a || a->n < 1 || a->n > SR_TN_GROUP_MAX) return SR_EINVAL;
  TnGroup G, Rd;
  G.n = Rd.n = a->n;
  int nb = 0, nr = 0;
  bool any_rows = false;
  for (int i = 0; i < a->n; ++i) {
    const sr_gemm_tn_args& p = a->p[i];
    const int rc = tn_check(&p);
    if (rc != SR_OK) return rc;
    if (tn_narrow(p.N, p.lddw)) return SR_EINVAL;
    const int tiles = (int)(sr_cdiv(p.N, 128) * sr_cdiv(p.K, 128));
    int rows_per_split = (int)sr_cdiv(p.R, p.splits);
    rows_per_split = (int)(sr_cdiv(rows_per_split, TBR) * TBR);
    G.p[i] = Rd.p[i] = p;
    G.rows_per_split[i] = Rd.rows_per_split[i] = rows_per_split;
    G.first[i] = nb; G.blocks[i] = p.R > 0 ? tiles * p.splits : 0;
    nb += (int)(sr_cdiv(G.blocks[i], 8) * 8);
    const int64_t total = (int64_t)p.N * p.lddw / 4 + (p.db ? p.N : 0);
    Rd.first[i] = nr; Rd.blocks[i] = sr_stream_grid(total, 256);
    nr += Rd.blocks[i];
    any_rows = any_rows || p.R > 0;
  }
  G.first[a->n] = nb; Rd.first[a->n] = nr;
  using Square = TnCfg<128, 128>;
  if (any_rows && nb > 0)
    hipLaunchKernelGGL(gemm_tn_group_kernel, dim3(nb), dim3(256), Square::kLdsFloats * sizeof(float), (hipStream_t)stream, G);
  hipLaunchKernelGGL(slab_reduce_group_kernel, dim3(nr), dim3(256), 0, (hipStream_t)stream, Rd);
  return sr_launch_status();
}
}

namespace {
__global__ __launch_bounds__(256) void pe_embed_kernel(const float* __restrict__ x, int64_t P, int L, const float* __restrict__ w,
                                                        const float* __restrict__ extra, int64_t ldextra, int E,
                                                        const int64_t* __restrict__ extra_index, int group,
                                                        float* __restrict__ out, int64_t ldo) {
  const int width = 3 + 6 * L + E;
  const int64_t total = P * ldo;
  for (int64_t i = (int64_t)blockIdx.x * blockDim.x + threadIdx.x; i < total; i += (int64_t)gridDim.x * blockDim.x) {
    const int64_t p = i / ldo;
    const int c = (int)(i % ldo);
    float v = 0.f, t3[3] = {0.f, 0.f, 0.f};
    if (c < 3) {
      v = x[p * 3 + c];
      t3[c] = 1.f;
    } else if (c < 3 + 6 * L) {
      const int k = (c - 3) / 6, r = (c - 3) % 6, comp = r % 3;
      const float f = (float)(1 << k);
      const float a = x[p * 3 + comp] * f;
      const float wk = w[2 * k + (r >= 3)];
      if (r < 3) { v = wk * sinf(a); t3[comp] = wk * f * cosf(a); }
      else { v = wk * cosf(a); t3[comp] = -wk * f * sinf(a); }
    } else if (c < width) {
      const int64_t src = extra_index ? extra_index[p] : p;
      v = extra[src * ldextra + (c - 3 - 6 * L)];
    }
    out[(p * group) * ldo + c] = v;
    if (group == 4) {
      out[(p * 4 + 1) * ldo + c] = t3[0];
      out[(p * 4 + 2) * ldo + c] = t3[1];
      out[(p * 4 + 3) * ldo + c] = t3[2];
    }
  }
}
}

extern "C" int sr_pe_embed(const float* x, int64_t P, int32_t L, const float* band_weights, const float* extra, int64_t ldextra,
                           int32_t E, const int64_t* extra_index, int32_t group, float* out, int64_t ldo, void* stream) {
  if (P < 0 || L < 0 || L > 16 || E < 0 || (group != 1 && group != 4) || ldo < 3 + 6 * L + E) return SR_EINVAL;
  if (P == 0) return SR_OK;
  if (!x || !out || (L > 0 && !band_weights) || (E > 0 && !extra)) return SR_EINVAL;
  sr_launch_stream(pe_embed_kernel, P * ldo, 256, stream, x, P, L, band_weights, extra, ldextra, E, extra_index, group, out, ldo);
  return sr_launch_status();
}

namespace {
__global__ __launch_bounds__(256) void pe_embed_bwd_kernel(const float* __restrict__ x, int64_t P, int L, const float* __restrict__ w,
                                                            int group, const float* __restrict__ gA0, int64_t ldg, float* __restrict__ xbar) {
  for (int64_t i = (int64_t)blockIdx.x * blockDim.x + threadIdx.x; i < P * 3; i += (int64_t)gridDim.x * blockDim.x) {
    const int64_t p = i / 3;
    const int c = (int)(i % 3);
    const float xv = x[i];
    const float* g0 = gA0 + (p * group) * ldg;
    const float* gt = group == 4 ? gA0 + (p * 4 + 1 + c) * ldg : nullptr;
    float acc = g0[c];
    for (int k = 0; k < L; ++k) {
      const float f = (float)(1 << k);
      float sn, cs;
      sincosf(xv * f, &sn, &cs);
      const float ws = w[2 * k], wc = w[2 * k + 1];
      const int is = 3 + 6 * k + c, ic = is + 3;
      acc += f * (ws * cs * g0[is] - wc * sn * g0[ic]);
      if (gt) acc -= f * f * (ws * sn * gt[is] + wc * cs * gt[ic]);
    }
    xbar[i] = acc;
  }
}
}

extern "C" int sr_pe_embed_bwd(const float* x, int64_t P, int32_t L, const float* band_weights, int32_t group, const float* gA0,
                               int64_t ldg, float* xbar, void* stream) {
  if (P < 0 || L < 0 || L > 16 || (group != 1 && group != 4) || ldg < 3 + 6 * L) return SR_EINVAL;
  if (P == 0) return SR_OK;
  if (!x || !gA0 || !xbar || (L > 0 && !band_weights)) return SR_EINVAL;
  sr_launch_stream(pe_embed_bwd_kernel, P * 3, 256, stream, x, P, L, band_weights, group, gA0, ldg, xbar);
  return sr_launch_status();
}
```

### selfreconcode_amd/mlp_engine.py

```python
import collections
import contextlib
import ctypes
import math
import os
import weakref
import torch

from . import _lib

ACT_NONE, ACT_SOFTPLUS100, ACT_RELU = _lib.SR_ACT_NONE, _lib.SR_ACT_SOFTPLUS100, _lib.SR_ACT_RELU
EPI_FWD, EPI_BWD = _lib.SR_EPI_FWD, _lib.SR_EPI_BWD

TN_SIDE_STREAM = True
GROUP_TN_BELOW = 16384
DEBUG_TN_DELAY_MS = int(os.environ.get("SR_DEBUG_TN_DELAY_MS", "0"))
_TN_STREAMS = {}
_TN_PENDING = set()
_DELAY_FLAG = {}

DEFERRED_PARAM_GRADS = False

_PACK_CACHE = {}
_ENTRY_BY_PTR = {}

_INPUT_GRADS_ONLY = False


def pad4(n):
    return (n + 3) // 4 * 4


class LayerSpec:
    __slots__ = ("K", "N", "act", "out_scale", "nfill")

    def __init__(self, K, N, act, out_scale=1.0, nfill=0):
        self.K, self.N, self.act, self.out_scale, self.nfill = K, N, act, float(out_scale), nfill


class MLPSpec:

    def __init__(self, layers, K0):
        self.layers = layers
        self.K0 = K0

    @staticmethod
    def sdf(multires=6, width=512, nlin=9, skip_in=(4,), d_out=257):
        K0 = 3 + 6 * multires
        layers = []
        k = K0
        for l in range(nlin):
            last = l == nlin - 1
            n = d_out if last else width
            if (l + 1) in skip_in:
                layers.append(LayerSpec(k, n - K0, ACT_SOFTPLUS100, 1.0 / math.sqrt(2.0), nfill=K0))
            else:
                layers.append(LayerSpec(k, n, ACT_NONE if last else ACT_SOFTPLUS100))
            k = n
        return MLPSpec(layers, K0)

    @staticmethod
    def relu_mlp(K0, widths):
        layers, k = [], K0
        for i, n in enumerate(widths):
            layers.append(LayerSpec(k, n, ACT_NONE if i == len(widths) - 1 else ACT_RELU))
            k = n
        return MLPSpec(layers, K0)


_GemmRecord = collections.namedtuple("_GemmRecord", "e0 e1 flop rows overlap N K mode group")


class _GemmProfile:

    def __init__(self):
        self.overlap = False
        self.reset(enabled=False)

    def reset(self, enabled, reserve=0):
        self.enabled = enabled
        self.records, self.chains, self.pool = [], [], []
        for _ in range(reserve if enabled else 0):
            e0, e1 = torch.cuda.Event(enable_timing=True), torch.cuda.Event(enable_timing=True)
            e0.record(); e1.record()
            self.pool.append((e0, e1))

    def pair(self):
        return self.pool.pop() if self.pool else (torch.cuda.Event(enable_timing=True), torch.cuda.Event(enable_timing=True))

    def launch(self, name, args, stream, timed=True, what=None, marks=None):
        if not (timed and self.enabled):
            _lib.call(name, ctypes.byref(args), stream)
            return
        e0, e1 = self.pair()
        e0.record()
        _lib.call(name, ctypes.byref(args), stream)
        e1.record()
        if marks is not None:
            marks.append((e0, e1) + what)
        else:
            rows, N, K, mode, group = what
            self.records.append(_GemmRecord(e0, e1, 2.0 * rows * N * K, rows, self.overlap, N, K, mode, group))

    def summary(self):
        if not self.records:
            return {"tflops": 0.0, "launches": 0, "avg_us": 0.0, "avg_flop": 0.0}
        torch.cuda.synchronize()
        for marks, live, overlap in self.chains:
            lv = live.tolist()
            for e0, e1, phase, fpr in marks:
                self.records.append(_GemmRecord(e0, e1, fpr * lv[phase], lv[phase], overlap, 0, 0, "chain", 1))
        self.chains = []
        times = [r.e0.elapsed_time(r.e1) for r in self.records]

        def rate(sel):
            f = sum(r.flop for r, t, k in zip(self.records, times, sel) if k)
            ms = sum(t for t, k in zip(times, sel) if k)
            n = sum(1 for k in sel if k)
            return (f / (ms * 1e-3) / 1e12 if ms > 0 else 0.0), n, (ms * 1e3 / n if n else 0.0), (f / n if n else 0.0)

        nt = [r.mode != "tn" for r in self.records]
        alone = [k and not r.overlap for k, r in zip(nt, self.records)]
        tf, n, us, fl = rate(alone)
        tf_all, n_all, us_all, _ = rate(nt)
        tf_big, n_big, _, _ = rate([a and r.rows >= 65536 for a, r in zip(alone, self.records)])
        tf_tn, n_tn, us_tn, _ = rate([not k for k in nt])
        self._times = times
        f_nt = float(sum(r.flop for r, k in zip(self.records, nt) if k))
        f_tn = float(sum(r.flop for r, k in zip(self.records, nt) if not k))
        return {"tflops": round(tf, 3), "launches": n, "avg_us": round(us, 3), "avg_flop": round(fl, 1), "tflops_large": round(tf_big, 3),
                "launches_large": n_big, "tflops_all": round(tf_all, 3), "launches_all": n_all, "avg_us_all": round(us_all, 3),
                "avg_flop_all": round(f_nt / max(n_all, 1), 1), "flops_total": f_nt, "flops_total_tn": f_tn,
                "tflops_tn": round(tf_tn, 3), "launches_tn": n_tn, "avg_us_tn": round(us_tn, 3)}

    def by_shape(self):
        if not self.records:
            return []
        times = getattr(self, "_times", None) or [r.e0.elapsed_time(r.e1) for r in self.records]
        acc = {}
        for r, t in zip(self.records, times):
            a = acc.setdefault((r.rows, r.N, r.K, r.mode, r.group, bool(r.overlap)), [0, 0.0, 0.0])
            a[0] += 1; a[1] += r.flop; a[2] += t
        rows = [{"M": k[0], "N": k[1], "K": k[2], "mode": k[3], "group": k[4], "overlap": k[5], "launches": v[0], "flop": v[1], "ms": round(v[2], 4),
                 "tflops": round(v[1] / (v[2] * 1e-3) / 1e12, 2) if v[2] > 0 else 0.0} for k, v in acc.items()]
        rows.sort(key=lambda r: -r["ms"])
        return rows


PROFILE = _GemmProfile()


def set_gemm_args(a, A, B, C, M, N, K, bias, group, act, mode, out_scale=1.0, aux=None, naux_fwd=0, nact_bwd=0, aux_scale=1.0, pitches=None):
    lda, ldb, ldc, ldaux = pitches or (A.stride(0), B.stride(0), C.stride(0), 0 if aux is None else aux.stride(0))
    a.A, a.lda, a.B, a.ldb, a.C, a.ldc = A.data_ptr(), lda, B.data_ptr(), ldb, C.data_ptr(), ldc
    a.M, a.N, a.K = M, N, K
    a.bias = _lib.ptr(bias)
    a.group, a.act, a.mode, a.out_scale = group, act, mode, out_scale
    a.aux, a.ldaux, a.naux_fwd, a.nact_bwd, a.aux_scale = _lib.ptr(aux), ldaux, naux_fwd, nact_bwd, aux_scale


def _gemm_nt(A, lda, B, ldb, C, ldc, M, N, K, bias, group, act, mode, out_scale=1.0, aux=None, ldaux=0, naux_fwd=0,
             nact_bwd=0, aux_scale=1.0):
    a = _lib.SrGemmArgs()
    set_gemm_args(a, A, B, C, M, N, K, bias, group, act, mode, out_scale, aux, naux_fwd, nact_bwd, aux_scale, (lda, ldb, ldc, ldaux))
    PROFILE.launch("sr_mlp_gemm_nt", a, _lib.stream_of(C), M >= 128 and N > 32, (M, N, K, mode, group))


_TnProblem = collections.namedtuple("_TnProblem", "Z ldz A lda R N K lddw group dW db accumulate")


def _tn_workspace(R, N, lddw):
    splits = ctypes.c_int32(0)
    ws = _lib.raw("sr_mlp_gemm_tn_workspace_floats")(R, N, lddw, ctypes.byref(splits))
    return max(int(ws), 1), splits.value


def _set_tn_args(a, Z, ldz, A, lda, R, N, K, lddw, group, dW, db, accumulate, partial, ws, splits):
    a.Z, a.ldz, a.A, a.lda, a.dW, a.lddw, a.partial = Z.data_ptr(), ldz, A.data_ptr(), lda, dW.data_ptr(), lddw, partial
    a.R, a.N, a.K, a.splits, a.accumulate = R, N, K, splits, 1 if accumulate else 0
    a.db, a.db_partial, a.group = db.data_ptr(), partial + 4 * ws, group


def _gemm_tn(Z, ldz, A, lda, R, N, K, lddw, group=1, dW=None, db=None, accumulate=False):
    ws, splits = _tn_workspace(R, N, lddw)
    if dW is None:
        dW = torch.empty((N, lddw), dtype=torch.float32, device=Z.device)
    partial = torch.empty((ws + splits * N,), dtype=torch.float32, device=Z.device)
    if db is None:
        db = torch.empty((N,), dtype=torch.float32, device=Z.device)
    a = _lib.SrGemmTnArgs()
    _set_tn_args(a, Z, ldz, A, lda, R, N, K, lddw, group, dW, db, accumulate, partial.data_ptr(), ws, splits)
    PROFILE.launch("sr_mlp_gemm_tn", a, _lib.stream_of(Z), R >= 128 and N > 32, (R, N, K, "tn", group))
    return dW, db


def _tn_is_narrow(N, lddw):
    return lddw <= 64 and N >= 256


def _gemm_tn_group(problems):
    problems = [_TnProblem(*p) for p in problems]
    g = _lib.SrGemmTnGroupArgs()
    g.n = len(problems)
    sizes, total = [], 0
    for p in problems:
        ws, splits = _tn_workspace(p.R, p.N, p.lddw)
        sizes.append((ws, splits, total))
        total += (ws + splits * p.N + 3) // 4 * 4
    partial = torch.empty((total,), dtype=torch.float32, device=problems[0].Z.device)
    for a, p, (ws, splits, off) in zip(g.p, problems, sizes):
        _set_tn_args(a, *p, partial.data_ptr() + 4 * off, ws, splits)
    _lib.call("sr_mlp_gemm_tn_group", ctypes.byref(g), _lib.stream_of(partial))


def _debug_delay(device, ms):
    f = _DELAY_FLAG.get(str(device))
    if f is None:
        f = _DELAY_FLAG[str(device)] = torch.zeros(2, dtype=torch.int32, device=device)
    _lib.call('sr_stream_flag_wait', f.data_ptr(), 0x40000000, 0, ms, torch.cuda.current_stream(device).cuda_stream)


def _tn_stream(device):
    key = str(device)
    st = _TN_STREAMS.get(key)
    if st is None:
        st = _TN_STREAMS[key] = torch.cuda.Stream(device=device)
    return st


def _launch_on_tn_stream(device, problems):
    main, side = torch.cuda.current_stream(device), _tn_stream(device)
    ready = torch.cuda.Event()
    ready.record(main)
    side.wait_event(ready)
    with torch.cuda.stream(side):
        if DEBUG_TN_DELAY_MS:
            _debug_delay(device, DEBUG_TN_DELAY_MS)
        if len(problems) == 1:
            p = problems[0]
            _gemm_tn(*p[:9], dW=p.dW, db=p.db, accumulate=p.accumulate)
        else:
            _gemm_tn_group(problems)
    for p in problems:
        p.Z.record_stream(side); p.A.record_stream(side)
    _TN_PENDING.add(str(device))


def join_weight_gradient_stream():
    for key in list(_TN_PENDING):
        st = _TN_STREAMS[key]
        torch.cuda.current_stream(st.device).wait_stream(st)
    _TN_PENDING.clear()


def _check_mat(t, name):
    if t.dtype != torch.float32 or not t.is_cuda or t.dim() != 2 or t.stride(1) != 1 or (t.stride(0) % 4) or (t.data_ptr() % 16):
        raise RuntimeError(f"mlp_engine: {name} must be a GPU fp32 matrix with unit column stride, row pitch % 4 == 0 "
                           f"and 16-byte alignment (got {tuple(t.shape)}, strides {t.stride()}, {t.dtype}, {t.device})")


def _bias_segments(b0, R, group):
    if b0 is None or b0.dim() != 2:
        return None
    S = b0.shape[0]
    if S < 1 or R % S or (R // S) % group or b0.stride(1) != 1:
        raise RuntimeError(f"mlp_engine: segmented first-layer bias {tuple(b0.shape)} does not divide {R} rows of group {group}")
    return S, R // S


def forward(spec, A0, Ws, bs, group):
    _check_mat(A0, "A0")
    R = A0.shape[0]
    acts, X = [], A0
    seg = _bias_segments(bs[0], R, group)
    with _lib.on_device(A0.device):
        for l, L in enumerate(spec.layers):
            _check_mat(Ws[l], f"W{l}")
            C = torch.empty((R, pad4(L.N + L.nfill)), dtype=torch.float32, device=A0.device)
            if l == 0 and seg is not None:
                S, rs = seg
                for s in range(S):
                    Xs, Cs = X[s * rs:(s + 1) * rs], C[s * rs:(s + 1) * rs]
                    _gemm_nt(Xs, X.stride(0), Ws[l], Ws[l].stride(0), Cs, C.stride(0), rs, L.N, L.K, bs[0][s], group, L.act, EPI_FWD,
                             out_scale=L.out_scale, aux=A0[s * rs:(s + 1) * rs] if L.nfill else None, ldaux=A0.stride(0), naux_fwd=L.nfill)
            else:
                _gemm_nt(X, X.stride(0), Ws[l], Ws[l].stride(0), C, C.stride(0), R, L.N, L.K, bs[l], group, L.act, EPI_FWD,
                         out_scale=L.out_scale, aux=A0 if L.nfill else None, ldaux=A0.stride(0), naux_fwd=L.nfill)
            acts.append(C)
            X = C
    return acts


_DW_GROUPED, _DW_SIDE, _DW_SINK, _DW_SEGMENTED, _DW_AUTOGRAD = range(5)


def _weight_gradient_route(l, L, Ws, bs, seg, grouped):
    segmented = l == 0 and seg is not None
    sink = None
    if DEFERRED_PARAM_GRADS and Ws is not None:
        if not segmented:
            sink = _deferred_sink(Ws[l], bs[l])
        if sink is None and not Ws[l].requires_grad:
            e = _ENTRY_BY_PTR.get(Ws[l].data_ptr())
            if e is not None and any(r() is not None and r().requires_grad for r in e.src):
                raise RuntimeError("mlp_engine: a packed weight handed out without autograd node (deferred mode) met a layer call "
                                   "that has no deferred sink (bias that is not the layer's own leaf parameter?): its gradient would be lost")
    if sink is None:
        return (_DW_SEGMENTED if segmented else _DW_AUTOGRAD), None
    if grouped is not None and not _tn_is_narrow(L.N, pad4(L.K)) and len(grouped) < _lib.SR_TN_GROUP_MAX:
        return _DW_GROUPED, sink
    if TN_SIDE_STREAM and not PROFILE.enabled:
        return _DW_SIDE, sink
    return _DW_SINK, sink


def reverse(spec, A0, WTs, acts, Ybar, group, need_input_grad=True, need_param_grad=True, Ws=None, bs=None):
    _check_mat(Ybar, "Ybar")
    R = A0.shape[0]
    nl = len(spec.layers)
    dWs, dbs = [None] * nl, [None] * nl
    A0bar_extra = None
    Zbar = Ybar
    A0bar = None
    seg = _bias_segments(bs[0], R, group) if bs is not None else None
    grouped = [] if (0 < R < GROUP_TN_BELOW and TN_SIDE_STREAM and not PROFILE.enabled) else None
    with _lib.on_device(A0.device):
        for l in range(nl - 1, -1, -1):
            L = spec.layers[l]
            X = A0 if l == 0 else acts[l - 1]
            if need_param_grad:
                route, sink = _weight_gradient_route(l, L, Ws, bs, seg, grouped)
                if sink is not None:
                    p = _TnProblem(Zbar, Zbar.stride(0), X, X.stride(0), R, L.N, L.K, pad4(L.K), group, *sink)
                    if route == _DW_GROUPED:
                        grouped.append(p)
                    elif route == _DW_SIDE:
                        _launch_on_tn_stream(A0.device, [p])
                    else:
                        _gemm_tn(*p[:9], dW=p.dW, db=p.db, accumulate=p.accumulate)
                elif route == _DW_SEGMENTED:
                    S, rs = seg
                    dWs[0] = torch.empty((L.N, pad4(L.K)), dtype=torch.float32, device=A0.device)
                    dbs[0] = torch.zeros((S, L.N), dtype=torch.float32, device=A0.device)
                    for s in range(S):
                        _gemm_tn(Zbar[s * rs:(s + 1) * rs], Zbar.stride(0), X[s * rs:(s + 1) * rs], X.stride(0), rs, L.N, L.K, pad4(L.K), group,
                                 dW=dWs[0], db=dbs[0][s], accumulate=s > 0)
                else:
                    dWs[l], dbs[l] = _gemm_tn(Zbar, Zbar.stride(0), X, X.stride(0), R, L.N, L.K, pad4(L.K), group)
            if l > 0:
                Pv = spec.layers[l - 1]
                Znew = torch.empty((R, pad4(L.K)), dtype=torch.float32, device=A0.device)
                _gemm_nt(Zbar, Zbar.stride(0), WTs[l], WTs[l].stride(0), Znew, Znew.stride(0), R, L.K, L.N, None, group, Pv.act,
                         EPI_BWD, out_scale=Pv.out_scale, aux=acts[l - 1], ldaux=acts[l - 1].stride(0), nact_bwd=Pv.N,
                         aux_scale=Pv.out_scale)
                if Pv.nfill and need_input_grad:
                    A0bar_extra = Znew[:, Pv.N:Pv.N + Pv.nfill]
                Zbar = Znew
            elif need_input_grad:
                A0bar = torch.empty((R, pad4(L.K)), dtype=torch.float32, device=A0.device)
                _gemm_nt(Zbar, Zbar.stride(0), WTs[0], WTs[0].stride(0), A0bar, A0bar.stride(0), R, L.K, L.N, None, 1, ACT_NONE,
                         EPI_FWD)
                if A0bar_extra is not None:
                    A0bar[:, :A0bar_extra.shape[1]] += A0bar_extra
        if grouped:
            _launch_on_tn_stream(A0.device, grouped)
    return A0bar, dWs, dbs


def transpose_padded(W, K):
    N = W.shape[0]
    WT = torch.zeros((K, pad4(N)), dtype=W.dtype, device=W.device)
    WT[:, :N] = W[:, :K].t()
    return WT


def pad_cols(t, width):
    if t.shape[1] == width and t.is_contiguous():
        return t
    return torch.nn.functional.pad(t, (0, width - t.shape[1]))


def rows_pad(a, width, b=None, pair=False):
    ref = a if a is not None else b
    R = ref.shape[0]
    if not pair and a.shape[1] == width and a.stride(1) == 1 and a.stride(0) % 4 == 0 and a.data_ptr() % 16 == 0:
        return a
    srcs = []
    for t in (a, b):
        if t is not None and (t.stride(1) != 1 or t.dtype != torch.float32):
            t = t.contiguous().float()
        srcs.append(t)
    a, b = srcs
    out = torch.empty((R * (2 if pair else 1), width), dtype=torch.float32, device=ref.device)
    with _lib.on_device(ref.device):
        _lib.call("sr_rows_pad", _lib.ptr(a), 0 if a is None else a.stride(0), 0 if a is None else min(a.shape[1], width),
                  _lib.ptr(b), 0 if b is None else b.stride(0), 0 if b is None else min(b.shape[1], width),
                  R, 2 if pair else 1, _lib.ptr(out), width, width, _lib.stream_of(ref))
    return out


def rows_frame_sum(X, index, n):
    P, E = X.shape
    if X.dtype != torch.float32 or X.stride(1) != 1:
        X = X.float().contiguous()
    index = index.contiguous()
    out = torch.empty((n, E), dtype=torch.float32, device=X.device)
    part = _lib.workspace("sr_rows_frame_sum_workspace_floats", P, E, n, device=X.device, dtype=torch.float32)
    with _lib.on_device(X.device):
        _lib.call("sr_rows_frame_sum", _lib.ptr(X), X.stride(0), P, E, _lib.ptr(index), n, _lib.ptr(part), _lib.ptr(out), _lib.stream_of(X))
    return out


@contextlib.contextmanager
def input_grads_only():
    global _INPUT_GRADS_ONLY
    prev = _INPUT_GRADS_ONLY
    _INPUT_GRADS_ONLY = True
    try:
        yield
    finally:
        _INPUT_GRADS_ONLY = prev


class MLPCoreFunction(torch.autograd.Function):

    @staticmethod
    def forward(ctx, spec, A0, *wb):
        nl = len(spec.layers)
        Ws, bs = list(wb[:nl]), list(wb[nl:])
        acts = forward(spec, A0, Ws, bs, 1)
        ctx.spec = spec
        ctx.save_for_backward(A0, *wb, *acts[:-1])
        ctx.set_materialize_grads(False)
        NL = spec.layers[-1].N
        out = acts[-1]
        return out if out.shape[1] == NL else out[:, :NL]

    @staticmethod
    def backward(ctx, ybar):
        if ybar is None:
            return (None,) * (2 + 2 * len(ctx.spec.layers))
        saved = ctx.saved_tensors
        nl = len(ctx.spec.layers)
        A0, wb, acts = saved[0], saved[1:1 + 2 * nl], saved[1 + 2 * nl:]
        need_par = any(ctx.needs_input_grad[2:]) and not _INPUT_GRADS_ONLY
        outs = MLPCoreBackward.apply(ctx.spec, ctx.needs_input_grad[1], need_par, A0, ybar, *wb, *acts)
        return (None,) + tuple(outs)


class MLPCoreBackward(torch.autograd.Function):

    @staticmethod
    def forward(ctx, spec, need_in, need_par, A0, ybar, *rest):
        nl = len(spec.layers)
        Ws, bs, acts = list(rest[:nl]), list(rest[nl:2 * nl]), list(rest[2 * nl:])
        NL = spec.layers[-1].N
        yb = rows_pad(ybar, pad4(NL))
        WTs = [transposed_of(Ws[l], spec.layers[l].K) for l in range(nl)]
        A0bar, dWs, dbs = reverse(spec, A0, WTs, acts, yb, 1, need_in, need_par, Ws, bs)
        ctx.spec = spec
        ctx.save_for_backward(A0, ybar, *Ws, *bs)
        ctx.set_materialize_grads(False)
        if not need_par:
            dWs, dbs = [None] * nl, [None] * nl
        if A0bar is not None and A0bar.shape[1] != A0.shape[1]:
            A0bar = rows_pad(A0bar[:, :spec.K0], A0.shape[1])
        return (A0bar,) + tuple(dWs) + tuple(dbs)

    @staticmethod
    def backward(ctx, U, *param_cots):
        spec = ctx.spec
        nl = len(spec.layers)
        if any(c is not None for c in param_cots):
            raise NotImplementedError("selfreconcode_amd: differentiating MLP parameter gradients again is not supported "
                                      "(the reference only differentiates input gradients, network.py:102-114)")
        n_in = 5 + 2 * nl + (nl - 1)
        if U is None:
            return (None,) * n_in
        saved = ctx.saved_tensors
        A0, ybar = saved[0], saved[1]
        Ws, bs = list(saved[2:2 + nl]), list(saved[2 + nl:2 + 2 * nl])
        NL = spec.layers[-1].N
        R = A0.shape[0]
        A0i = rows_pad(A0, A0.shape[1], U, pair=True)
        acts2 = forward(spec, A0i, Ws, bs, 2)
        ydot = acts2[-1].view(R, 2, -1)[:, 1, :NL]
        ybi = rows_pad(None, pad4(NL), ybar, pair=True)
        WTs = [transposed_of(Ws[l], spec.layers[l].K) for l in range(nl)]
        need_in = ctx.needs_input_grad[3]
        need_par = any(ctx.needs_input_grad[5:5 + 2 * nl])
        A0bar2, dWs, dbs = reverse(spec, A0i, WTs, acts2, ybi, 2, need_in, need_par, Ws, bs)
        gA0 = A0bar2.view(R, 2, -1)[:, 0, :] if A0bar2 is not None else None
        if gA0 is not None and gA0.shape[1] != A0.shape[1]:
            gA0 = rows_pad(gA0[:, :spec.K0], A0.shape[1])
        return (None, None, None, gA0, ydot.contiguous()) + tuple(dWs) + tuple(dbs) + (None,) * (nl - 1)


def mlp_apply(spec, A0, Ws, bs):
    return MLPCoreFunction.apply(spec, A0, *Ws, *bs)


class _Pack:
    __slots__ = ("W", "WT", "norms", "sig", "src", "bias_param", "dW", "db", "bias", "fresh", "dirty")

    def __init__(self, W, WT, norms):
        self.W, self.WT, self.norms, self.sig, self.src = W, WT, norms, None, ()
        self.dW = self.db = self.bias = self.bias_param = None
        self.fresh, self.dirty = True, False


def _sig(*ts):
    return tuple((t.data_ptr(), t._version, tuple(t.shape)) for t in ts)


def _lin_params(lin):
    return (lin.weight_v, lin.weight_g) if hasattr(lin, "weight_g") else (lin.weight, None)


def _lin_sig(v, g):
    return _sig(v) if g is None else _sig(v, g)


def _raise_if_dirty(e):
    if e.dirty:
        raise RuntimeError("mlp_engine: parameters changed while deferred gradients were pending; call flush_param_grads() "
                           "before the optimizer step")


def _drop_entry(key):
    e = _PACK_CACHE.pop(key, None)
    if e is not None:
        _ENTRY_BY_PTR.pop(e.W.data_ptr(), None)


def _pack_entry(key, sig, build, owner=None):
    e = _PACK_CACHE.get(key)
    if e is None and owner is not None:
        weakref.finalize(owner, _drop_entry, key)
    if e is None or e.sig != sig:
        if e is not None:
            _raise_if_dirty(e)
            _drop_entry(key)
        e = build()
        e.sig = sig
        _PACK_CACHE[key] = e
        _ENTRY_BY_PTR[e.W.data_ptr()] = e
    return e


class PackWeightNorm(torch.autograd.Function):
    @staticmethod
    def forward(ctx, v, g):
        K = v.shape[1]

        def build():
            with torch.no_grad():
                w, norms = torch._weight_norm_interface(v, g, 0)
                W = pad_cols(w, pad4(K)).contiguous()
                return _Pack(W, transpose_padded(W, K), norms)
        e = _pack_entry(id(v), _sig(v, g), build, owner=v)
        e.src = (weakref.ref(v), weakref.ref(g))
        ctx.save_for_backward(v, g, e.norms)
        ctx.set_materialize_grads(False)
        return e.W.detach()

    @staticmethod
    def backward(ctx, gW):
        if gW is None:
            return None, None
        v, g, norms = ctx.saved_tensors
        gv, gg = torch.ops.aten._weight_norm_interface_backward(gW[:, :v.shape[1]].contiguous(), v, g, norms, 0)
        return gv, gg


class PackPlain(torch.autograd.Function):
    @staticmethod
    def forward(ctx, w):
        K = w.shape[1]

        def build():
            with torch.no_grad():
                W = pad_cols(w, pad4(K)).contiguous()
                if W.data_ptr() == w.data_ptr():
                    W = W.clone()
                return _Pack(W, transpose_padded(W, K), None)
        e = _pack_entry(id(w), _sig(w), build, owner=w)
        e.src = (weakref.ref(w),)
        ctx.K = K
        ctx.set_materialize_grads(False)
        return e.W.detach()

    @staticmethod
    def backward(ctx, gW):
        return None if gW is None else gW[:, :ctx.K]


def refresh_packs(lins):
    if not lins or not _lin_params(lins[0])[0].is_cuda:
        return
    stale = []
    for lin in lins:
        v, g = _lin_params(lin)
        e = _PACK_CACHE.get(id(v))
        if e is None:
            continue
        sig = _lin_sig(v, g)
        if e.sig != sig:
            _raise_if_dirty(e)
            if e.W.shape != (v.shape[0], pad4(v.shape[1])):
                continue
            stale.append((e, v, g, sig))
    for i in range(0, len(stale), _lib.SR_PACK_MAX_LAYERS):
        chunk = stale[i:i + _lib.SR_PACK_MAX_LAYERS]
        t = _lib.SrPackTable()
        t.nlayers = len(chunk)
        for j, (e, v, g, sig) in enumerate(chunk):
            L = t.layer[j]
            vv = v.detach()
            if not vv.is_contiguous():
                vv = vv.contiguous()
            L.v, L.g = _lib.ptr(vv), (0 if g is None else _lib.ptr(g.detach().contiguous()))
            L.W, L.WT, L.norms = _lib.ptr(e.W), _lib.ptr(e.WT), (0 if g is None else _lib.ptr(e.norms))
            L.N, L.K, L.ldw, L.ldwt = v.shape[0], v.shape[1], e.W.stride(0), e.WT.stride(0)
        with _lib.on_device(chunk[0][1].device), torch.no_grad():
            _lib.call("sr_pack_weights", ctypes.byref(t), _lib.stream_of(chunk[0][1]))
        for e, v, g, sig in chunk:
            e.sig = sig
        torch.autograd.graph.increment_version([t for e, _, _, _ in chunk for t in (e.W, e.WT, e.norms) if t is not None])


def pack_linear(lin):
    v, g = _lin_params(lin)
    if DEFERRED_PARAM_GRADS:
        e = _PACK_CACHE.get(id(v))
        b = lin.bias
        if e is not None and e.sig == _lin_sig(v, g) and e.src and b is not None and b.is_leaf and b.requires_grad:
            e.bias_param = b
            return e.W
    W = PackPlain.apply(v) if g is None else PackWeightNorm.apply(v, g)
    e = _ENTRY_BY_PTR.get(W.data_ptr())
    if e is not None:
        e.bias_param = lin.bias
    return W


def packed_weights_of(module, nlayers):
    d = module.__dict__
    mods = module._modules
    lins = [mods["lin" + str(l)] for l in range(nlayers)]
    params = []
    for lin in lins:
        P = lin._parameters
        v = P.get('weight_v')
        if v is not None:
            params.append(v); params.append(P['weight_g'])
        else:
            params.append(P['weight'])
        b = P.get('bias')
        if b is not None:
            params.append(b)
    key = (DEFERRED_PARAM_GRADS,) + tuple((id(p), p.data_ptr(), p._version, p.requires_grad) for p in params)
    hit = d.get('_sr_packs')
    if hit is not None and hit[0] == key:
        return list(hit[1]), list(hit[2])
    refresh_packs(lins)
    Ws, bs = [pack_linear(lin) for lin in lins], [lin.bias for lin in lins]
    if DEFERRED_PARAM_GRADS and all(W.grad_fn is None and not W.requires_grad and W.data_ptr() in _ENTRY_BY_PTR for W in Ws):
        d['_sr_packs'] = (key, list(Ws), list(bs))
    else:
        d.pop('_sr_packs', None)
    return Ws, bs


def transposed_of(W, K):
    e = _ENTRY_BY_PTR.get(W.data_ptr())
    if e is not None:
        WT = e.WT
        if WT.shape == (K, pad4(W.shape[0])):
            return WT
        if W.stride(0) == e.W.stride(0) and W.shape[0] <= e.W.shape[0] and K <= WT.shape[0] and pad4(W.shape[0]) <= WT.shape[1]:
            return WT[:K, :pad4(W.shape[0])]
    return transpose_padded(W, K)


def set_deferred_param_grads(flag):
    global DEFERRED_PARAM_GRADS
    flush_param_grads()
    DEFERRED_PARAM_GRADS = bool(flag)


def _deferred_sink(W, b):
    e = _ENTRY_BY_PTR.get(W.data_ptr())
    if e is None or b is None or not b.requires_grad or W.shape[0] > e.W.shape[0] or W.stride(0) != e.W.stride(0):
        return None
    n, full = W.shape[0], W.shape[0] == e.W.shape[0]
    if full:
        if not b.is_leaf:
            return None
    else:
        base = e.bias_param
        if base is None or not base.is_leaf or not base.requires_grad or b.data_ptr() != base.data_ptr():
            return None
        b = base
    if e.dW is None:
        e.dW = torch.empty_like(e.W)
        e.db = torch.empty((e.W.shape[0],), dtype=torch.float32, device=e.W.device)
        e.fresh = True
    if e.fresh and not full:
        e.dW.zero_(); e.db.zero_()
        e.fresh = False
    accumulate = not e.fresh
    e.fresh = False
    e.dirty = True
    e.bias = b
    return e.dW[:n], e.db[:n], accumulate


def flush_param_grads(only=None):
    todo = [e for e in _PACK_CACHE.values() if e.dirty and (only is None or id(e.src[0]()) in only)]
    if not todo:
        return
    join_weight_gradient_stream()
    for i in range(0, len(todo), _lib.SR_PACK_MAX_LAYERS):
        chunk = todo[i:i + _lib.SR_PACK_MAX_LAYERS]
        t = _lib.SrUnpackTable()
        t.nlayers = len(chunk)
        outs = []
        for j, e in enumerate(chunk):
            L = t.layer[j]
            src = tuple(r() for r in e.src)
            v = src[0]
            g = src[1] if len(src) == 2 else None
            acc = v.grad is not None and (g is None or g.grad is not None)
            gv = v.grad if acc else torch.empty_like(v, memory_format=torch.contiguous_format)
            gg = None
            if g is not None:
                gg = g.grad if acc else torch.empty_like(g, memory_format=torch.contiguous_format)
            if acc and (not gv.is_contiguous() or (gg is not None and not gg.is_contiguous())):
                acc = False
                gv = torch.empty_like(v, memory_format=torch.contiguous_format)
                gg = None if g is None else torch.empty_like(g, memory_format=torch.contiguous_format)
            vd = v.detach()
            if not vd.is_contiguous():
                vd = vd.contiguous()
            L.dW, L.lddw = _lib.ptr(e.dW), e.dW.stride(0)
            L.v, L.g, L.norms = _lib.ptr(vd), (0 if g is None else _lib.ptr(g.detach().contiguous())), (0 if g is None else _lib.ptr(e.norms))
            L.gv, L.gg, L.N, L.K, L.accumulate = _lib.ptr(gv), _lib.ptr(gg), v.shape[0], v.shape[1], 1 if acc else 0
            b = e.bias
            fold_bias = b.grad is not None and b.grad.is_contiguous() and b.grad.dtype == torch.float32
            L.db, L.gb = (_lib.ptr(e.db), _lib.ptr(b.grad)) if fold_bias else (0, 0)
            outs.append((e, v, g, gv, gg, acc, vd, fold_bias))
        dev = chunk[0].W.device
        with _lib.on_device(dev), torch.no_grad():
            _lib.call("sr_unpack_grads", ctypes.byref(t), torch.cuda.current_stream(dev).cuda_stream)
        for e, v, g, gv, gg, acc, _, fold_bias in outs:
            if not acc:
                v.grad = gv if v.grad is None else v.grad.add_(gv)
                if g is not None:
                    g.grad = gg if g.grad is None else g.grad.add_(gg)
            b = e.bias
            if fold_bias:
                torch.autograd.graph.increment_version(b.grad)
            elif b.grad is None:
                b.grad = e.db
                e.db = torch.empty_like(e.db)
            else:
                b.grad.add_(e.db)
            e.fresh = True
            e.dirty = False
```

### selfreconcode_amd/model/Deformer.py

```python
import ctypes
import os

import numpy as np
import torch
import torch.nn as nn
import torch.nn.functional as F

from .. import _lib
from .Embedder import embed_rows
from ..MCAcc.grid_sampler_mine import GridSamplerMine3dFunction
from ..mlp_engine import MLPSpec, mlp_apply, pad_cols, pad4, pack_linear
from ..utils.utils import resolve_band_weights


BATCH_FRAMES = True
HOIST_FRAME_CODE = True


_EYE3 = {}


def _eye3(device):
    e = _EYE3.get(device)
    if e is None:
        e = _EYE3[device] = torch.eye(3).to(device)
        if e.is_cuda:
            torch.cuda.current_stream(device).synchronize()
    return e


class CompositeDeformer(nn.Module):
    def __init__(self, deformers):
        super().__init__()
        self.N = len(deformers)
        self.defs = nn.ModuleList(deformers)

    def forward(self, ps, conds, batch_inds=None, **kwargs):
        assert self.N == len(conds)
        out = ps
        for cond, deformer in zip(conds, self.defs):
            out = deformer(out, cond, batch_inds, **kwargs)
        return out


class MLPTranslator(nn.Module):

    def __init__(self, feature_vector_size, multires, weight_norm=False):
        super().__init__()
        assert multires > 0
        dims = [3 + 6 * multires + feature_vector_size, 512, 512, 512, 512, 3]
        self.feature_vector_size = feature_vector_size
        self.multires = multires
        self.num_layers = len(dims)
        for l in range(0, self.num_layers - 1):
            lin = nn.Linear(dims[l], dims[l + 1])
            if weight_norm:
                print('MLPTranslator:weight norm can influence weight initialization, can not produce small weights as '
                      'initialization. Now do not use weight_norm')
            if l == self.num_layers - 2:
                torch.nn.init.normal_(lin.weight, mean=0., std=0.001)
                torch.nn.init.constant_(lin.bias, 0.)
            setattr(self, "lin" + str(l), lin)
        self.spec = MLPSpec.relu_mlp(dims[0], dims[1:])
        self.offset = None

    def packed_weights(self):
        from ..mlp_engine import packed_weights_of
        return packed_weights_of(self, len(self.spec.layers))

    def hoisted_first_layer(self, conds, frames=None):
        npe = 3 + 6 * self.multires
        W0 = self.lin0.weight
        Bf = conds.reshape(-1, self.feature_vector_size) @ W0[:, npe:].t() + self.lin0.bias
        if frames is not None and Bf.shape[0] != frames:
            raise ValueError(f"MLPTranslator: {Bf.shape[0]} condition codes for a batch of {frames} frames")
        W0p = pad_cols(W0[:, :npe], pad4(npe))
        spec = getattr(self, "_spec_pe", None)
        if spec is None:
            spec = self._spec_pe = MLPSpec.relu_mlp(npe, [L.N for L in self.spec.layers])
        return spec, W0p, Bf

    def forward(self, ps, conds, batch_inds=None, **kwargs):
        ratio = kwargs['ratio']['deformerRatio']
        ws = resolve_band_weights(self.multires, ratio)
        if batch_inds is None and HOIST_FRAME_CODE and ps.dim() == 3:
            spec, W0p, Bf = self.hoisted_first_layer(conds, ps.shape[0])
            Ws, bs = self.packed_weights()
            if BATCH_FRAMES:
                A0 = embed_rows(ps.reshape(-1, 3), self.multires, ws)
                self.offset = mlp_apply(spec, A0, [W0p] + Ws[1:], [Bf] + bs[1:]).view(ps.shape[0], ps.shape[1], 3)
                return ps[..., :3] + self.offset
            outs = []
            for p_f, B_f in zip(ps.unbind(0), Bf.unbind(0)):
                A0 = embed_rows(p_f, self.multires, ws)
                outs.append(mlp_apply(spec, A0, [W0p] + Ws[1:], [B_f] + bs[1:]))
            self.offset = torch.stack(outs, 0)
            return ps[..., :3] + self.offset
        if batch_inds is not None:
            flat, index, seg = ps, batch_inds, 0
        else:
            nb, nv = ps.shape[0], ps.shape[1]
            flat = ps.reshape(-1, 3)
            index = torch.arange(nb, device=ps.device).repeat_interleave(nv)
            seg = nv
        A0 = embed_rows(flat, self.multires, ws, extra=conds.reshape(-1, self.feature_vector_size), extra_index=index, segment=seg)
        Ws, bs = self.packed_weights()
        x = mlp_apply(self.spec, A0, Ws, bs)
        if batch_inds is not None:
            self.offset = x
            return ps[..., :3] + x
        self.offset = x.view(ps.shape[0], ps.shape[1], 3)
        return ps[..., :3] + self.offset


def getTranslatorNet(device, conf):
    return MLPTranslator(conf.get_int('condlen'), multires=conf.get_int('multires')).to(device)


def batch_rodrigues(theta):
    angle = torch.norm(theta + 1e-8, p=2, dim=1, keepdim=True)
    axis = theta / angle
    half = angle * 0.5
    q = torch.cat([torch.cos(half), torch.sin(half) * axis], dim=1)
    q = q / q.norm(p=2, dim=1, keepdim=True)
    w, x, y, z = q[:, 0], q[:, 1], q[:, 2], q[:, 3]
    w2, x2, y2, z2 = w * w, x * x, y * y, z * z
    wx, wy, wz, xy, xz, yz = w * x, w * y, w * z, x * y, x * z, y * z
    return torch.stack([w2 + x2 - y2 - z2, 2 * xy - 2 * wz, 2 * wy + 2 * xz,
                        2 * wz + 2 * xy, w2 - x2 + y2 - z2, 2 * yz - 2 * wx,
                        2 * xz - 2 * wy, 2 * wx + 2 * yz, w2 - x2 - y2 + z2], dim=1).view(-1, 3, 3)


def _tree_levels(parents):
    depth = [0] * len(parents)
    for i in range(1, len(parents)):
        depth[i] = depth[int(parents[i])] + 1
    return [[i for i in range(len(parents)) if depth[i] == d] for d in range(1, max(depth) + 1)]


class LBSkinner(nn.Module):

    def __init__(self, ws, bmins, bmaxs, Js, parents, init_pose=None, align_corners=False):
        super().__init__()

        def as_row(v):
            if isinstance(v, list):
                return torch.tensor(v, dtype=torch.float).view(1, 3)
            if isinstance(v, np.ndarray):
                return torch.from_numpy(v.astype(np.float32)).view(1, 3)
            return v.view(1, 3)
        self.register_buffer('b_min', as_row(bmins))
        self.register_buffer('b_max', as_row(bmaxs))
        ws = torch.from_numpy(ws.astype(np.float32)) if isinstance(ws, np.ndarray) else ws.to(torch.float)
        assert ws.dim() == 5 and ws.shape[0] == 1 and ws.shape[1] == 24
        self.register_buffer('ws', ws.contiguous(memory_format=torch.channels_last_3d))
        assert align_corners is False
        self.align_corners = align_corners
        self.register_buffer('Js', Js.view(24, 3).float())
        self.parents = [int(p) for p in parents]
        self._levels = _tree_levels(self.parents)
        if init_pose is None:
            raise NotImplementedError("the reference always builds the skinner with an init pose (network.py:843,851)")
        if isinstance(init_pose, np.ndarray):
            init_pose = torch.from_numpy(init_pose.astype(np.float32))
        if init_pose.numel() == 24 * 3:
            self.init_pose_inverse(batch_rodrigues(init_pose.view(-1, 3)).view(24, 3, 3), self.Js)
        else:
            self.register_buffer('init_pose', init_pose.view(24, 4, 4))

    def _apply(self, fn, *a, **k):
        out = super()._apply(fn, *a, **k)
        if not self.ws.is_contiguous(memory_format=torch.channels_last_3d):
            self.ws = self.ws.contiguous(memory_format=torch.channels_last_3d)
        return out

    def init_pose_inverse(self, init_pose, Js):
        R, T = [init_pose[0]], [Js[0]]
        for i in range(1, 24):
            pa = self.parents[i]
            R.append(R[pa] @ init_pose[i])
            T.append(R[pa] @ (Js[i] - Js[pa]) + T[pa])
        inv = torch.zeros(24, 4, 4)
        for i in range(24):
            inv[i, :3, :3] = R[i].t()
            inv[i, :3, 3] = -(R[i].t() @ T[i])
            inv[i, 3, 3] = 1.
        self.register_buffer('init_pose', inv)

    def _chain(self, poses):
        B = poses.shape[0]
        R = batch_rodrigues(poses.reshape(-1, 3)).view(B, 24, 3, 3)
        rel = self.Js.clone()
        rel[1:] = self.Js[1:] - self.Js[self.parents[1:]]
        local = torch.cat([torch.cat([R, rel.view(1, 24, 3, 1).expand(B, 24, 3, 1)], 3),
                           torch.cat([rel.new_zeros(3), rel.new_ones(1)]).view(1, 1, 1, 4).expand(B, 24, 1, 4)], 2)
        G = [None] * 24
        G[0] = local[:, 0]
        for level in self._levels:
            pa = torch.stack([G[self.parents[i]] for i in level], 1)
            prod = pa @ local[:, level]
            for n, i in enumerate(level):
                G[i] = prod[:, n]
        return torch.stack(G, 1)

    def _buffers_key(self):
        return tuple((t.data_ptr(), t._version) for t in (self.Js, self.init_pose, self.b_min, self.b_max))

    def _host_consts(self):
        key = self._buffers_key()
        if getattr(self, "_hc_key", None) != key:
            js = (ctypes.c_float * 72)(*self.Js.detach().cpu().view(-1).tolist())
            pa = (ctypes.c_int32 * 24)(*[max(p, 0) if i else 0 for i, p in enumerate(self.parents)])
            ip = (ctypes.c_float * 384)(*self.init_pose.detach().cpu().view(-1).tolist())
            self._hc = (js, pa, ip)
            self._box = (self.b_min.view(-1).tolist(), self.b_max.view(-1).tolist())
            self._hc_key = key
        return self._hc

    def _box_consts(self):
        self._host_consts()
        return self._box

    def posed_chain(self, poses):
        if poses.is_cuda:
            return _PosedChain.apply(self, poses)
        G = self._chain(poses)
        return G, G @ self.init_pose.view(1, 24, 4, 4)

    def posed_transforms(self, poses):
        return self.posed_chain(poses)[1]

    def posedSkeleton(self, conds):
        poses, trans = conds
        assert poses.shape[0] == trans.shape[0]
        return self.posed_chain(poses)[0][:, :, :3, 3]

    def fill_lbs_fields(self, a, A, trans):
        A12 = A[:, :, :3, :].contiguous()
        vol = self.ws.permute(0, 2, 3, 4, 1)
        assert vol.is_contiguous()
        a.A, a.trans, a.nframes = _lib.ptr(A12), _lib.ptr(trans), A.shape[0]
        a.vol, a.D, a.H, a.W = _lib.ptr(vol), vol.shape[1], vol.shape[2], vol.shape[3]
        box = self._box_consts()
        for i in range(3):
            a.bmin[i], a.bmax[i] = box[0][i], box[1][i]
        return A12, vol

    def _lbs_args(self, flat, A, trans, batch_inds, ppf, tp=None):
        a = _lib.SrLbsArgs()
        keep = self.fill_lbs_fields(a, A, trans)
        a.p, a.tp, a.P = _lib.ptr(flat), _lib.ptr(tp), flat.shape[0]
        a.batch_inds, a.points_per_frame = _lib.ptr(batch_inds), ppf
        return a, keep

    def fused(self, ps, A, trans, batch_inds=None, with_jac=False, tps=None):
        flat = ps.reshape(-1, 3).contiguous()
        P = flat.shape[0]
        tr = trans.contiguous()
        tp = None if tps is None else tps.reshape(-1, 3).contiguous()
        ppf = 0 if batch_inds is not None else (ps.shape[1] if ps.dim() == 3 else P)
        a, keep = self._lbs_args(flat, A, tr, batch_inds, ppf, tp)
        y = torch.empty_like(flat)
        jac = torch.empty((P, 3, 3), device=flat.device) if with_jac else None
        a.y, a.jac = _lib.ptr(y), _lib.ptr(jac)
        _lib.launch("sr_lbs_fwd", flat, ctypes.byref(a))
        return y.view(ps.shape), jac

    def forward(self, ps, conds, batch_inds=None, **kwargs):
        if type(ps) == list:
            tps, ps = ps
        else:
            tps = ps
        poses, trans = conds
        batch_size = poses.shape[0]
        assert batch_size == trans.shape[0]
        A = self.posed_transforms(poses)
        needs_graph = torch.is_grad_enabled() and (ps.requires_grad or tps.requires_grad or poses.requires_grad or trans.requires_grad)
        if not needs_graph:
            y, _ = self.fused(ps, A, trans, batch_inds, False, None if tps is ps else tps)
            return y
        if tps is ps:
            flat = ps.reshape(-1, 3)
            ppf = 0 if batch_inds is not None else ps.shape[1]
            y = _FusedLBS.apply(self, flat, A, trans, batch_inds, ppf)
            return y.view(ps.shape)
        return self._composite(ps, tps, A, trans, batch_inds)

    def _composite(self, ps, tps, A, trans, batch_inds):
        batch_size = A.shape[0]
        nps = 2. * (tps.reshape(-1, 3) - self.b_min) / (self.b_max - self.b_min) - 1.
        w = GridSamplerMine3dFunction.apply(self.ws, nps.reshape(1, 1, 1, -1, 3)).view(24, -1).transpose(0, 1)
        A12 = A[:, :, :3, :].reshape(batch_size, 24, 12)
        if batch_inds is None:
            nb, pnum, _ = ps.shape
            assert nb == batch_size
            T = torch.matmul(w.view(nb, pnum, 24), A12).view(nb, pnum, 3, 4)
            return (T[..., :3] @ ps.unsqueeze(-1)).squeeze(-1) + T[..., 3] + trans.view(-1, 1, 3)
        p = ps.reshape(-1, 3)
        Tall = (w @ A12.permute(1, 0, 2).reshape(24, batch_size * 12)).view(-1, batch_size, 12)
        T = torch.gather(Tall, 1, batch_inds.view(-1, 1, 1).expand(-1, 1, 12)).view(-1, 3, 4)
        return (T[..., :3] @ p.unsqueeze(-1)).squeeze(-1) + T[..., 3] + trans[batch_inds]

    def fused_backward(self, flat, A, batch_inds, ppf, ybar, need_p, need_A, need_t, Jbar=None):
        N, dev = A.shape[0], flat.device
        a, keep = self._lbs_args(flat, A, None, batch_inds, ppf)
        cots = [None if ybar is None else ybar.contiguous().float()] + ([] if Jbar is None else [Jbar.contiguous().float()])
        pbar = torch.empty_like(flat) if need_p else None
        Abar = torch.empty((N, 24, 12), device=dev) if need_A else None
        tbar = torch.empty((N, 3), device=dev) if (need_t and ybar is not None) else None
        part = _lib.workspace("sr_lbs_bwd_workspace_floats", flat.shape[0], N, device=dev, dtype=torch.float32)
        _lib.launch("sr_lbs_bwd" if Jbar is None else "sr_lbs_jac_bwd", flat, ctypes.byref(a), *cots, pbar, Abar, tbar, part)
        return pbar, Abar, tbar


def _frame_major(flat, A, batch_inds):
    return flat if batch_inds is not None else flat.view(A.shape[0], -1, 3)


def _cotangent_4x4(Abar):
    return None if Abar is None else F.pad(Abar.view(-1, 24, 3, 4), (0, 0, 0, 1))


class _PosedChain(torch.autograd.Function):
    @staticmethod
    def forward(ctx, skin, poses):
        p = poses.detach().contiguous().float().view(-1, 24, 3)
        B = p.shape[0]
        G = torch.empty((B, 24, 4, 4), dtype=torch.float32, device=p.device)
        A = torch.empty_like(G)
        js, pa, ip = skin._host_consts()
        _lib.launch("sr_lbs_chain_fwd", p, p, B, js, pa, ip, G, A)
        ctx.skin = skin
        ctx.save_for_backward(p)
        ctx.pshape = poses.shape
        ctx.set_materialize_grads(False)
        return G, A

    @staticmethod
    def backward(ctx, Gbar, Abar):
        if Gbar is None and Abar is None:
            return None, None
        (p,) = ctx.saved_tensors
        js, pa, ip = ctx.skin._host_consts()
        out = torch.empty_like(p)
        gb = None if Gbar is None else Gbar.contiguous().float()
        ab = None if Abar is None else Abar.contiguous().float()
        _lib.launch("sr_lbs_chain_bwd", p, p, p.shape[0], js, pa, ip, ab, gb, out)
        return None, out.view(ctx.pshape)


class _FusedLBS(torch.autograd.Function):

    @staticmethod
    def forward(ctx, skin, flat, A, trans, batch_inds, ppf):
        flat = flat.contiguous()
        y, _ = skin.fused(_frame_major(flat, A, batch_inds), A, trans, batch_inds, False, None)
        ctx.skin, ctx.ppf = skin, ppf
        ctx.save_for_backward(flat, A, trans, batch_inds)
        return y.reshape(-1, 3)

    @staticmethod
    def backward(ctx, ybar):
        flat, A, trans, batch_inds = ctx.saved_tensors
        skin = ctx.skin
        need_p, need_A, need_t = ctx.needs_input_grad[1], ctx.needs_input_grad[2], ctx.needs_input_grad[3]
        if torch.is_grad_enabled():
            ps = _frame_major(flat, A, batch_inds)
            y2 = skin._composite(ps, ps, A, trans, batch_inds).reshape(-1, 3)
            ins = [t for t, n in ((flat, need_p), (A, need_A), (trans, need_t)) if n]
            gs = list(torch.autograd.grad(y2, ins, ybar, create_graph=True, allow_unused=True))
            out = [gs.pop(0) if n else None for n in (need_p, need_A, need_t)]
            return None, out[0], out[1], out[2], None, None
        pbar, Abar, tbar = skin.fused_backward(flat, A, batch_inds, ctx.ppf, ybar, need_p, need_A, need_t)
        return None, pbar, _cotangent_4x4(Abar), tbar, None, None


class _LBSValueJacobian(torch.autograd.Function):

    @staticmethod
    def forward(ctx, skin, q, A, trans, batch_inds, ppf):
        flat = q.reshape(-1, 3).contiguous().float()
        y, J = skin.fused(_frame_major(flat, A, batch_inds), A, trans, batch_inds, True, None)
        ctx.skin, ctx.ppf = skin, ppf
        ctx.save_for_backward(flat, A, batch_inds)
        ctx.set_materialize_grads(False)
        return y.reshape(-1, 3), J

    @staticmethod
    def backward(ctx, ybar, Jbar):
        flat, A, batch_inds = ctx.saved_tensors
        skin = ctx.skin
        if ybar is None and Jbar is None:
            return (None,) * 6
        need_q, need_A, need_t = ctx.needs_input_grad[1], ctx.needs_input_grad[2], ctx.needs_input_grad[3]
        Jb = torch.zeros((flat.shape[0], 3, 3), device=flat.device) if Jbar is None else Jbar
        qbar, Abar, tbar = skin.fused_backward(flat, A, batch_inds, ctx.ppf, ybar, need_q, need_A, need_t, Jb)
        return None, qbar, _cotangent_4x4(Abar), tbar, None, None


def deformer_value_jacobian(deformer, ps, defconds, batch_inds, ratio):
    tr, skin = deformer.defs[0], deformer.defs[1]
    d_cond, (poses, trans) = defconds[0], defconds[1]
    q, Jq = translator_value_jacobian(tr, ps, d_cond, batch_inds, ratio)
    A = skin.posed_transforms(poses)
    y, Jl = _LBSValueJacobian.apply(skin, q, A, trans, batch_inds, 0)
    from ..utils.utils import small_matmul
    return y, small_matmul(Jl, Jq)


def is_fused_composite(deformer):
    return (isinstance(deformer, CompositeDeformer) and deformer.N == 2 and isinstance(deformer.defs[0], MLPTranslator)
            and isinstance(deformer.defs[1], LBSkinner))


class TranslatorValueJacobian(torch.autograd.Function):

    @staticmethod
    def forward(ctx, tr, ratio, x, conds, index, segment, spec, *wb):
        from .. import mlp_engine as me
        from .Embedder import band_weight_tensor
        spec = spec or tr.spec
        nl = len(spec.layers)
        Ws, bs = list(wb[:nl]), list(wb[nl:])
        flat = x.reshape(-1, 3).contiguous().float()
        P = flat.shape[0]
        wt, _ = band_weight_tensor(resolve_band_weights(tr.multires, ratio), tr.multires, flat.device)
        E = 0 if conds is None else tr.feature_vector_size
        ldo = me.pad4(3 + 6 * tr.multires + E)
        A0 = torch.empty((P * 4, ldo), dtype=torch.float32, device=flat.device)
        cd = None if conds is None else conds.reshape(-1, E).contiguous().float()
        with _lib.on_device(flat.device):
            _lib.launch("sr_pe_embed", flat, flat, P, tr.multires, wt, cd, 0 if cd is None else cd.stride(0), E, index, 4, A0, ldo)
            acts = me.forward(spec, A0, Ws, bs, 4)
        out = acts[-1].view(P, 4, -1)[:, :, :3]
        d = flat + out[:, 0]
        J = out[:, 1:4].transpose(1, 2) + _eye3(flat.device)
        ctx.tr, ctx.wt, ctx.segment, ctx.n_extra, ctx.xshape, ctx.spec, ctx.E = tr, wt, segment, 0 if cd is None else cd.shape[0], x.shape, spec, E
        ctx.set_materialize_grads(False)
        ctx.save_for_backward(flat, index, A0, *wb, *acts[:-1])
        return d.view(x.shape), J

    @staticmethod
    def backward(ctx, dbar, Jbar):
        from .. import mlp_engine as me
        tr, spec = ctx.tr, ctx.spec
        nl = len(spec.layers)
        saved = ctx.saved_tensors
        flat, index, A0 = saved[0], saved[1], saved[2]
        wb, acts = saved[3:3 + 2 * nl], list(saved[3 + 2 * nl:])
        Ws = list(wb[:nl])
        P = flat.shape[0]
        if dbar is None and Jbar is None:
            return (None,) * (7 + 2 * nl)
        ybar = torch.zeros((P, 4, 4), dtype=torch.float32, device=flat.device)
        if dbar is not None:
            ybar[:, 0, :3] = dbar.reshape(-1, 3)
        if Jbar is not None:
            ybar[:, 1:4, :3] = Jbar.transpose(1, 2)
        WTs = [me.transposed_of(Ws[l], spec.layers[l].K) for l in range(nl)]
        acts_full = acts + [None]
        need_par = any(ctx.needs_input_grad[7:])
        need_x = ctx.needs_input_grad[2]
        need_in = need_x or (ctx.needs_input_grad[3] and ctx.E > 0)
        A0bar, dWs, dbs = me.reverse(spec, A0, WTs, acts_full, ybar.view(P * 4, 4), 4, need_in, need_par, Ws, list(wb[nl:]))
        if not need_par:
            dWs, dbs = [None] * nl, [None] * nl
        xbar = None
        if need_x:
            xbar = torch.empty_like(flat)
            _lib.launch("sr_pe_embed_bwd", flat, flat, P, tr.multires, ctx.wt, 4, A0bar, A0bar.stride(0), xbar)
            if dbar is not None:
                xbar = xbar + dbar.reshape(-1, 3)
            xbar = xbar.view(ctx.xshape)
        gcond = None
        if ctx.needs_input_grad[3] and ctx.E:
            E = ctx.E
            ge = A0bar.view(P, 4, -1)[:, 0, 3 + 6 * tr.multires:3 + 6 * tr.multires + E]
            if ctx.segment:
                gcond = ge.reshape(ctx.n_extra, ctx.segment, E).sum(1)
            else:
                gcond = (me.rows_frame_sum(ge, index, ctx.n_extra) if ctx.n_extra <= 32
                         else torch.zeros((ctx.n_extra, E), dtype=ge.dtype, device=ge.device).index_add(0, index, ge))
        return (None, None, xbar, gcond, None, None, None) + tuple(dWs) + tuple(dbs)


def translator_value_jacobian(tr, ps, conds, batch_inds, ratio):
    r = ratio['deformerRatio'] if isinstance(ratio, dict) else ratio
    if batch_inds is not None:
        index, seg = batch_inds, 0
    else:
        index = torch.arange(ps.shape[0], device=ps.device).repeat_interleave(ps.shape[1])
        seg = ps.shape[1]
    Ws, bs = tr.packed_weights()
    if batch_inds is None and HOIST_FRAME_CODE and ps.dim() == 3:
        spec, W0p, Bf = tr.hoisted_first_layer(conds, ps.shape[0])
        if BATCH_FRAMES:
            return TranslatorValueJacobian.apply(tr, r, ps.contiguous(), None, None, 0, spec, W0p, *Ws[1:], Bf, *bs[1:])
        ds_, Js_ = [], []
        for p_f, B_f in zip(ps.unbind(0), Bf.unbind(0)):
            d_f, J_f = TranslatorValueJacobian.apply(tr, r, p_f.contiguous(), None, None, 0, spec, W0p, *Ws[1:], B_f, *bs[1:])
            ds_.append(d_f); Js_.append(J_f)
        return torch.stack(ds_, 0), torch.cat(Js_, 0)
    return TranslatorValueJacobian.apply(tr, r, ps, conds, index, seg, None, *Ws, *bs)


def smooth_weights(weights, times=3):
    from .. import ops
    _lib.require_gpu(weights)
    if weights.dim() != 5 or weights.shape[0] != 1:
        raise ValueError(f"smooth_weights: weights [1,nj,D,H,W] expected, got {tuple(weights.shape)}")
    if int(times) <= 0:
        return weights
    return ops.lbsw_smooth(weights.detach()[0].contiguous().float(), times).unsqueeze(0)


def _three(v):
    if torch.is_tensor(v):
        v = v.detach().cpu().numpy()
    return [float(x) for x in np.asarray(v, dtype=np.float32).reshape(3)]


def compute_lbswField(bmins, bmaxs, resolutions, smpl_verts, smpl_ws, align_corners=False, mean_neighbor=5, smooth_times=30):
    from .. import ops
    _lib.require_gpu(smpl_verts, smpl_ws)
    field = ops.lbsw_knn_blend(smpl_verts, smpl_ws, _three(bmins), _three(bmaxs), resolutions, mean_neighbor, align_corners)
    return ops.lbsw_smooth(field, smooth_times, consume=True).unsqueeze(0)


LBS_BOX_MARGIN = (0.15, 0.15, 0.20)


def initialLBSkinner(gender, shape, pose, resolution, bmins=None, bmaxs=None, smpl=None):
    from ..smpl_pytorch import getSMPL
    _lib.require_gpu(shape, pose)
    smpl = (smpl if smpl is not None else getSMPL(gender)).to(shape.device)
    Js = smpl.skeleton(shape.view(1, -1), True)[0]
    verts = smpl(shape.view(1, -1), pose.view(1, 24, 3), True)[0][0]
    skinner = initial_lbs_skinner(verts, smpl.weight[0], Js.view(24, 3), smpl.parents, pose.view(24, 3), resolution, bmins, bmaxs)
    return skinner, verts, smpl.faces_tensor.to(verts.device)


def initial_lbs_skinner(verts, skin_weights, Js, parents, init_pose, resolution, bmins=None, bmaxs=None):
    _lib.require_gpu(verts, skin_weights)
    if bmins is None or bmaxs is None:
        margin = np.array(LBS_BOX_MARGIN, dtype=np.float32)
        bmins = (verts.min(0)[0].cpu().numpy() - margin).tolist()
        bmaxs = (verts.max(0)[0].cpu().numpy() + margin).tolist()
    ws = compute_lbswField(bmins, bmaxs, resolution, verts, skin_weights, align_corners=False, mean_neighbor=30, smooth_times=30)
    pose = torch.from_numpy(init_pose.astype(np.float32)) if isinstance(init_pose, np.ndarray) else init_pose.detach().float().cpu()
    skinner = LBSkinner(ws, _three(bmins), _three(bmaxs), torch.as_tensor(Js).detach().float().cpu(), np.asarray(parents), init_pose=pose,
                        align_corners=False)
    return skinner.to(verts.device)
```

Before: 23.51.

## Add tangent-only plane-layout reverse pass for deformer Jacobian backward

When only the Jacobian output carries a gradient and no input gradient is needed, the deformer backward now runs a dedicated reverse pass. It stores the three tangent planes as separate contiguous row blocks and skips the value row that carries no gradient. The NT and TN GEMM kernels gain a PLANES template mode that offsets A/C/Z pointers per plane and strides the interleaved activations, and bias-gradient partials are skipped in that mode. The aim is to avoid computing and storing a quarter of the rows (the zero value row) in the backward GEMMs. The cost is extra kernel template instantiations and a more restricted, special-cased code path.

New measurement: 23.18. 0.986x the previous value.

```diff
diff --git a/include/selfrecon_hip.h b/include/selfrecon_hip.h
--- a/include/selfrecon_hip.h
+++ b/include/selfrecon_hip.h
@@ -72,6 +72,7 @@
   int32_t naux_fwd;
   int32_t nact_bwd;
   float aux_scale;
+  int32_t planes;
 } sr_gemm_args;
 int sr_mlp_gemm_nt(const sr_gemm_args* host_args, void* stream);
 int sr_mlp_gemm_nt_tile(int32_t M, int32_t ncols, int32_t* bm_out, int32_t* bn_out);
@@ -93,6 +94,7 @@
   float* partial;
   int32_t R, N, K, splits, accumulate;
   float* db; float* db_partial; int32_t group;
+  int32_t planes;
 } sr_gemm_tn_args;
 int64_t sr_mlp_gemm_tn_workspace_floats(int32_t R, int32_t N, int64_t lddw, int32_t* host_splits_out);
 int sr_mlp_gemm_tn(const sr_gemm_tn_args* host_args, void* stream);
diff --git a/selfreconcode_amd/csrc/mlp_gemm.hip b/selfreconcode_amd/csrc/mlp_gemm.hip
--- a/selfreconcode_amd/csrc/mlp_gemm.hip
+++ b/selfreconcode_amd/csrc/mlp_gemm.hip
@@ -259,20 +259,32 @@
 }
 
 struct NoProbe { __device__ __forceinline__ void operator()(int) const {} };
-template <int WM, int WN, int TM, int TN, bool KTAIL = true, class Probe = NoProbe>
-__device__ __forceinline__ void gemm_nt_tile(const sr_gemm_args& g, int wg, float* __restrict__ smem, Probe probe = Probe()) {
+template <int WM, int WN, int TM, int TN, bool KTAIL = true, bool PLANES = false, class Probe = NoProbe>
+__device__ __forceinline__ void gemm_nt_tile(const sr_gemm_args& g_launch, int wg, float* __restrict__ smem, Probe probe = Probe()) {
   using C_ = Cfg<WM, WN, TM, TN>;
   auto As = [&](int buf) -> float* { return smem + buf * (C_::BM * LDSP); };
   auto Bs = [&](int buf) -> float* { return smem + 2 * C_::BM * LDSP + buf * (C_::BN * LDSP); };
 
-  const int tiles_n = (g.N + g.naux_fwd + C_::BN - 1) / C_::BN;
-  const int tiles_m = (g.M + C_::BM - 1) / C_::BM;
+  const int tiles_n = (g_launch.N + g_launch.naux_fwd + C_::BN - 1) / C_::BN;
+  const int tiles_mp = (g_launch.M + C_::BM - 1) / C_::BM;
+  const int tiles_m = PLANES ? tiles_mp * g_launch.planes : tiles_mp;
   const int nwg = tiles_m * tiles_n;
   {
     const int q = nwg / 8, r = nwg % 8, xcd = wg % 8, loc = wg / 8;
     wg = (xcd < r ? xcd * (q + 1) : r * (q + 1) + (xcd - r) * q) + loc;
   }
-  const int tn = wg % tiles_n, tm = wg / tiles_n;
+  const int tn = wg % tiles_n;
+  int tm = wg / tiles_n;
+  sr_gemm_args g_plane;
+  if constexpr (PLANES) {
+    const int plane = tm / tiles_mp;
+    tm -= plane * tiles_mp;
+    g_plane = g_launch;
+    g_plane.A += (int64_t)plane * g_launch.M * g_launch.lda;
+    g_plane.C += (int64_t)plane * g_launch.M * g_launch.ldc;
+    g_plane.ldaux = g_launch.ldaux * (g_launch.planes + 1);
+  }
+  const sr_gemm_args& g = PLANES ? g_plane : g_launch;
   const int m0 = tm * C_::BM, n0 = tn * C_::BN;
 
   const int lane = threadIdx.x & 63, wave = threadIdx.x >> 6;
@@ -363,7 +375,11 @@
 
   float* stage = smem + wave * (TM * 32 * (TN * 32 + 4));
   const bool interior = m0 + C_::BM <= g.M && n0 + C_::BN <= (g.mode == SR_EPI_FWD ? g.N : (g.nact_bwd < g.N ? g.nact_bwd : g.N));
-  if (interior) {
+  if constexpr (PLANES) {
+    if (!interior) epilogue<WM, WN, TM, TN, 1>(g, acc, m0, n0, wm, wn, li, kh, stage);
+    else if (g.act == SR_ACT_RELU) epilogue_interior<WM, WN, TM, TN, 1, SR_EPI_BWD, SR_ACT_RELU>(g, acc, m0, n0, wm, wn, li, kh, stage);
+    else epilogue_interior<WM, WN, TM, TN, 1, SR_EPI_BWD, SR_ACT_NONE>(g, acc, m0, n0, wm, wn, li, kh, stage);
+  } else if (interior) {
     if (g.mode == SR_EPI_FWD) {
       switch (g.group) {
         case 1: epilogue_interior_act<WM, WN, TM, TN, 1, SR_EPI_FWD>(g, acc, m0, n0, wm, wn, li, kh, stage); break;
@@ -387,10 +403,10 @@
   probe(2);
 }
 
-template <int WM, int WN, int TM, int TN, bool KTAIL>
+template <int WM, int WN, int TM, int TN, bool KTAIL, bool PLANES>
 __global__ __launch_bounds__(WM * WN * 64) __attribute__((amdgpu_waves_per_eu(2))) void gemm_nt_kernel(sr_gemm_args g) {
   extern __shared__ __attribute__((aligned(16))) float smem[];
-  gemm_nt_tile<WM, WN, TM, TN, KTAIL>(g, blockIdx.x, smem);
+  gemm_nt_tile<WM, WN, TM, TN, KTAIL, PLANES>(g, blockIdx.x, smem);
 }
 
 
@@ -406,18 +422,31 @@
   static constexpr int WN = XW / 64;
 };
 
-template <int ZW, int XW>
-__device__ __forceinline__ void gemm_tn_body(const sr_gemm_tn_args& g, int rows_per_split, int bid, int nblocks, float* __restrict__ tn_smem) {
+template <int ZW, int XW, bool PLANES = false>
+__device__ __forceinline__ void gemm_tn_body(const sr_gemm_tn_args& g_launch, int rows_per_split, int bid, int nblocks, float* __restrict__ tn_smem) {
   using C = TnCfg<ZW, XW>;
   auto Zs = [&](int buf) -> float* { return tn_smem + buf * C::kZ; };
   auto Xs = [&](int buf) -> float* { return tn_smem + 2 * C::kZ + buf * C::kX; };
-  const int tiles_k = (g.K + XW - 1) / XW;
-  const int tiles_n = (g.N + ZW - 1) / ZW;
+  const int tiles_k = (g_launch.K + XW - 1) / XW;
+  const int tiles_n = (g_launch.N + ZW - 1) / ZW;
   int vb = bid;
   if ((nblocks & 7) == 0) vb = (bid & 7) * (nblocks >> 3) + (bid >> 3);
   const int tile = vb % (tiles_k * tiles_n), split = vb / (tiles_k * tiles_n);
   const int n0 = (tile / tiles_k) * ZW, k0 = (tile % tiles_k) * XW;
-  const int r_begin = split * rows_per_split;
+  int slab = split;
+  sr_gemm_tn_args g_plane;
+  if constexpr (PLANES) {
+    const int per_plane = g_launch.splits / g_launch.planes;
+    const int plane = split / per_plane;
+    slab -= plane * per_plane;
+    g_plane = g_launch;
+    g_plane.Z += (int64_t)plane * g_launch.R * g_launch.ldz;
+    g_plane.A += (int64_t)(1 + plane) * g_launch.lda;
+    g_plane.lda = g_launch.lda * (g_launch.planes + 1);
+    g_plane.db_partial = nullptr;
+  }
+  const sr_gemm_tn_args& g = PLANES ? g_plane : g_launch;
+  const int r_begin = slab * rows_per_split;
   const int r_end = min(g.R, r_begin + rows_per_split);
   const int lane = threadIdx.x & 63, wave = threadIdx.x >> 6;
   const int wm = wave / C::WN, wn = wave % C::WN, li = lane & 31, kh = lane >> 5;
@@ -517,7 +546,7 @@
     }
   };
 
-  const bool do_bias = g.db_partial != nullptr && k0 == 0;
+  const bool do_bias = !PLANES && g.db_partial != nullptr && k0 == 0;
   const float wodd = g.group == 4 ? 0.f : 1.f;
   float bsum0 = 0.f, bsum1 = 0.f;
   auto bias_half = [&](const float (&z0)[HS], const float (&z1)[HS]) {
@@ -600,10 +629,10 @@
     }
 }
 
-template <int ZW, int XW>
+template <int ZW, int XW, bool PLANES>
 __global__ __launch_bounds__(256) __attribute__((amdgpu_waves_per_eu(2))) void gemm_tn_kernel(sr_gemm_tn_args g, int rows_per_split) {
   extern __shared__ __attribute__((aligned(16))) float tn_smem[];
-  gemm_tn_body<ZW, XW>(g, rows_per_split, blockIdx.x, gridDim.x, tn_smem);
+  gemm_tn_body<ZW, XW, PLANES>(g, rows_per_split, blockIdx.x, gridDim.x, tn_smem);
 }
 
 struct TnGroup {
@@ -626,7 +655,7 @@
 
 __device__ __forceinline__ void slab_reduce_body(const float* __restrict__ partial, float* __restrict__ dW, int N,
                                                  int K, int64_t lddw, int splits, int accumulate,
-                                                 const float* __restrict__ db_partial, float* __restrict__ db, int bid, int nblocks) {
+                                                 const float* __restrict__ db_partial, float* __restrict__ db, int db_splits, int bid, int nblocks) {
   const int64_t total = (int64_t)N * lddw;
   const int64_t quads = total >> 2;
   const int64_t all = quads + (db ? N : 0);
@@ -657,7 +686,7 @@
     } else {
       const int n = (int)(i - quads);
       float s = 0.f;
-      for (int p = 0; p < splits; ++p) s += db_partial[(int64_t)p * N + n];
+      for (int p = 0; p < db_splits; ++p) s += db_partial[(int64_t)p * N + n];
       db[n] = (accumulate ? db[n] : 0.f) + s;
     }
   }
@@ -665,8 +694,8 @@
 
 __global__ __launch_bounds__(256) void slab_reduce_kernel(const float* __restrict__ partial, float* __restrict__ dW, int N,
                                                            int K, int64_t lddw, int splits, int accumulate,
-                                                           const float* __restrict__ db_partial, float* __restrict__ db) {
-  slab_reduce_body(partial, dW, N, K, lddw, splits, accumulate, db_partial, db, blockIdx.x, gridDim.x);
+                                                           const float* __restrict__ db_partial, float* __restrict__ db, int db_splits) {
+  slab_reduce_body(partial, dW, N, K, lddw, splits, accumulate, db_partial, db, db_splits, blockIdx.x, gridDim.x);
 }
 
 __global__ __launch_bounds__(256) void slab_reduce_group_kernel(TnGroup G) {
@@ -675,14 +704,15 @@
   const int bid = blockIdx.x - G.first[i];
   if (bid >= G.blocks[i]) return;
   const sr_gemm_tn_args& g = G.p[i];
-  slab_reduce_body(g.partial, g.dW, g.N, g.K, g.lddw, g.R > 0 ? g.splits : 0, g.accumulate, g.db_partial, g.db, bid, G.blocks[i]);
-}
-
-}
-
-static void nt_tile_choice(int M, int ncols, int* bm, int* bn) {
+  const int splits = g.R > 0 ? g.splits : 0;
+  slab_reduce_body(g.partial, g.dW, g.N, g.K, g.lddw, splits, g.accumulate, g.db_partial, g.db, splits, bid, G.blocks[i]);
+}
+
+}
+
+static void nt_tile_choice(int M, int ncols, int* bm, int* bn, int planes = 1) {
   auto cost = [&](int tm, int tn, double eff) {
-    const int64_t wgs = sr_cdiv(M, tm) * sr_cdiv(ncols, tn);
+    const int64_t wgs = planes * sr_cdiv(M, tm) * sr_cdiv(ncols, tn);
     return (double)sr_cdiv(wgs, 256) * tm * tn / eff;
   };
   if (ncols <= 32) {
@@ -712,22 +742,32 @@
   if (a->mode == SR_EPI_FWD && a->naux_fwd > 0 && !a->aux) return SR_EINVAL;
   if (a->M == 0) return SR_OK;
   if (a->M % a->group) return SR_EINVAL;
+  if (a->planes) {
+    const int64_t limit = 1ll << 32;
+    if ((a->planes != 1 && a->planes != 3) || a->group != 1 || a->mode != SR_EPI_BWD || a->nact_bwd < a->N) return SR_EINVAL;
+    if ((a->act != SR_ACT_RELU && a->act != SR_ACT_NONE) || (a->act == SR_ACT_RELU && !a->aux) || (a->ldaux & 3)) return SR_EINVAL;
+    if (a->M * a->lda * 4 >= limit || a->M * a->ldc * 4 >= limit || a->M * (a->planes + 1) * a->ldaux * 4 >= limit) return SR_EINVAL;
+  }
+  const int planes = a->planes ? a->planes : 1;
   const int ncols = a->N + (a->mode == SR_EPI_FWD ? a->naux_fwd : 0);
   sr_gemm_args g = *a;
   if (g.mode != SR_EPI_FWD) g.naux_fwd = 0;
 #define SR_NT_LAUNCH(WM, WN, TM, TN)                                                                                        \
   do {                                                                                                                      \
     using C_ = Cfg<WM, WN, TM, TN>;                                                                                         \
-    const int nwg = (int)(sr_cdiv(g.M, C_::BM) * sr_cdiv(ncols, C_::BN));                                                   \
-    if (g.K % BK)                                                                                                           \
-      hipLaunchKernelGGL((gemm_nt_kernel<WM, WN, TM, TN, true>), dim3(nwg), dim3(C_::kThreads), C_::kLdsFloats * sizeof(float), \
-                         (hipStream_t)stream, g);                                                                           \
-    else                                                                                                                    \
-      hipLaunchKernelGGL((gemm_nt_kernel<WM, WN, TM, TN, false>), dim3(nwg), dim3(C_::kThreads), C_::kLdsFloats * sizeof(float), \
-                         (hipStream_t)stream, g);                                                                           \
+    const int nwg = (int)(planes * sr_cdiv(g.M, C_::BM) * sr_cdiv(ncols, C_::BN));                                          \
+    const dim3 grid(nwg), block(C_::kThreads);                                                                              \
+    const size_t lds = C_::kLdsFloats * sizeof(float);                                                                      \
+    if (g.planes) {                                                                                                         \
+      if (g.K % BK) hipLaunchKernelGGL((gemm_nt_kernel<WM, WN, TM, TN, true, true>), grid, block, lds, (hipStream_t)stream, g);   \
+      else hipLaunchKernelGGL((gemm_nt_kernel<WM, WN, TM, TN, false, true>), grid, block, lds, (hipStream_t)stream, g);     \
+    } else {                                                                                                                \
+      if (g.K % BK) hipLaunchKernelGGL((gemm_nt_kernel<WM, WN, TM, TN, true, false>), grid, block, lds, (hipStream_t)stream, g);  \
+      else hipLaunchKernelGGL((gemm_nt_kernel<WM, WN, TM, TN, false, false>), grid, block, lds, (hipStream_t)stream, g);    \
+    }                                                                                                                       \
   } while (0)
   int bm = 0, bn = 0;
-  nt_tile_choice(g.M, ncols, &bm, &bn);
+  nt_tile_choice(g.M, ncols, &bm, &bn, planes);
   switch (bm * 1024 + bn) {
     case 32 * 1024 + 32: SR_NT_LAUNCH(1, 1, 1, 1); break;
     case 64 * 1024 + 32: SR_NT_LAUNCH(2, 1, 1, 1); break;
@@ -766,7 +806,7 @@
     if (a->nprob[l] < 1 || a->nprob[l] > 2) return SR_EINVAL;
     for (int p = 0; p < a->nprob[l]; ++p) {
       const sr_gemm_args& g = a->g[l][p];
-      if (!g.A || !g.B || !g.C || g.N <= 0 || g.K <= 0 || g.group != a->m_mul) return SR_EINVAL;
+      if (!g.A || !g.B || !g.C || g.N <= 0 || g.K <= 0 || g.group != a->m_mul || g.planes) return SR_EINVAL;
       if ((g.lda & 3) || (g.ldb & 3) || (g.ldc & 3) || ((uintptr_t)g.A & 15) || ((uintptr_t)g.B & 15) || ((uintptr_t)g.C & 15)) return SR_EINVAL;
       if (g.mode != SR_EPI_FWD && g.mode != SR_EPI_BWD) return SR_EINVAL;
       if (g.mode == SR_EPI_BWD && g.naux_fwd != 0) return SR_EINVAL;
@@ -797,39 +837,45 @@
   return (int64_t)splits * N * lddw;
 }
 
-int sr_mlp_gemm_tn(const sr_gemm_tn_args* a, void* stream) {
-  if (!a || !a->dW || !a->partial || a->R < 0 || a->N <= 0 || a->K <= 0 || a->splits < 1) return SR_EINVAL;
-  if (a->R > 0 && (!a->Z || !a->A)) return SR_EINVAL;
-  if ((a->ldz & 3) || (a->lda & 3) || ((uintptr_t)a->Z & 15) || ((uintptr_t)a->A & 15) || a->lddw < a->K) return SR_EINVAL;
-  if ((a->lddw & 3) || ((uintptr_t)a->dW & 15) || ((uintptr_t)a->partial & 15)) return SR_EINVAL;
-  if ((a->db != nullptr) != (a->db_partial != nullptr) || (a->db && a->group < 1)) return SR_EINVAL;
-  const bool narrow = tn_narrow(a->N, a->lddw);
-  const int tiles = narrow ? (int)sr_cdiv(a->N, 256) : (int)(sr_cdiv(a->N, 128) * sr_cdiv(a->K, 128));
-  int rows_per_split = (int)sr_cdiv(a->R, a->splits);
-  rows_per_split = (int)(sr_cdiv(rows_per_split, TBR) * TBR);
-  if (a->R > 0) {
-    using Narrow = TnCfg<256, 64>;
-    using Square = TnCfg<128, 128>;
-    if (narrow)
-      hipLaunchKernelGGL((gemm_tn_kernel<256, 64>), dim3(tiles * a->splits), dim3(256), Narrow::kLdsFloats * sizeof(float), (hipStream_t)stream, *a,
-                         rows_per_split);
-    else
-      hipLaunchKernelGGL((gemm_tn_kernel<128, 128>), dim3(tiles * a->splits), dim3(256), Square::kLdsFloats * sizeof(float), (hipStream_t)stream, *a,
-                         rows_per_split);
-  }
-  const int64_t total = (int64_t)a->N * a->lddw / 4 + (a->db ? a->N : 0);
-  sr_launch_stream(slab_reduce_kernel, total, 256, stream, a->partial, a->dW, a->N, a->K, a->lddw, a->R > 0 ? a->splits : 0, a->accumulate, a->db_partial,
-                   a->db);
-  return sr_launch_status();
-}
-
 static int tn_check(const sr_gemm_tn_args* a) {
   if (!a || !a->dW || !a->partial || a->R < 0 || a->N <= 0 || a->K <= 0 || a->splits < 1) return SR_EINVAL;
   if (a->R > 0 && (!a->Z || !a->A)) return SR_EINVAL;
   if ((a->ldz & 3) || (a->lda & 3) || ((uintptr_t)a->Z & 15) || ((uintptr_t)a->A & 15) || a->lddw < a->K) return SR_EINVAL;
   if ((a->lddw & 3) || ((uintptr_t)a->dW & 15) || ((uintptr_t)a->partial & 15)) return SR_EINVAL;
+  if (a->planes) {
+    const int64_t limit = 1ll << 32;
+    if ((a->planes != 1 && a->planes != 3) || a->splits % a->planes) return SR_EINVAL;
+    if (a->R * a->ldz * 4 >= limit || a->R * (a->planes + 1) * a->lda * 4 >= limit) return SR_EINVAL;
+    return SR_OK;
+  }
   if ((a->db != nullptr) != (a->db_partial != nullptr) || (a->db && a->group < 1)) return SR_EINVAL;
   return SR_OK;
+}
+
+int sr_mlp_gemm_tn(const sr_gemm_tn_args* a, void* stream) {
+  const int rc = tn_check(a);
+  if (rc != SR_OK) return rc;
+  const bool narrow = tn_narrow(a->N, a->lddw);
+  const int tiles = narrow ? (int)sr_cdiv(a->N, 256) : (int)(sr_cdiv(a->N, 128) * sr_cdiv(a->K, 128));
+  int rows_per_split = (int)sr_cdiv(a->R, a->planes ? a->splits / a->planes : a->splits);
+  rows_per_split = (int)(sr_cdiv(rows_per_split, TBR) * TBR);
+  if (a->R > 0) {
+    const dim3 grid(tiles * a->splits), block(256);
+    const size_t narrow_lds = TnCfg<256, 64>::kLdsFloats * sizeof(float), square_lds = TnCfg<128, 128>::kLdsFloats * sizeof(float);
+    if (a->planes) {
+      if (narrow) hipLaunchKernelGGL((gemm_tn_kernel<256, 64, true>), grid, block, narrow_lds, (hipStream_t)stream, *a, rows_per_split);
+      else hipLaunchKernelGGL((gemm_tn_kernel<128, 128, true>), grid, block, square_lds, (hipStream_t)stream, *a, rows_per_split);
+    } else {
+      if (narrow) hipLaunchKernelGGL((gemm_tn_kernel<256, 64, false>), grid, block, narrow_lds, (hipStream_t)stream, *a, rows_per_split);
+      else hipLaunchKernelGGL((gemm_tn_kernel<128, 128, false>), grid, block, square_lds, (hipStream_t)stream, *a, rows_per_split);
+    }
+  }
+  const int splits = a->R > 0 ? a->splits : 0;
+  float* db = a->planes && a->accumulate ? nullptr : a->db;
+  const int64_t total = (int64_t)a->N * a->lddw / 4 + (db ? a->N : 0);
+  sr_launch_stream(slab_reduce_kernel, total, 256, stream, a->partial, a->dW, a->N, a->K, a->lddw, splits, a->accumulate, a->db_partial, db,
+                   a->planes ? 0 : splits);
+  return sr_launch_status();
 }
 
 int sr_mlp_gemm_tn_group(const sr_gemm_tn_group_args* a, void* stream) {
@@ -842,7 +888,7 @@
     const sr_gemm_tn_args& p = a->p[i];
     const int rc = tn_check(&p);
     if (rc != SR_OK) return rc;
-    if (tn_narrow(p.N, p.lddw)) return SR_EINVAL;
+    if (tn_narrow(p.N, p.lddw) || p.planes) return SR_EINVAL;
     const int tiles = (int)(sr_cdiv(p.N, 128) * sr_cdiv(p.K, 128));
     int rows_per_split = (int)sr_cdiv(p.R, p.splits);
     rows_per_split = (int)(sr_cdiv(rows_per_split, TBR) * TBR);
diff --git a/selfreconcode_amd/mlp_engine.py b/selfreconcode_amd/mlp_engine.py
--- a/selfreconcode_amd/mlp_engine.py
+++ b/selfreconcode_amd/mlp_engine.py
@@ -159,37 +159,56 @@
 
 
 def _gemm_nt(A, lda, B, ldb, C, ldc, M, N, K, bias, group, act, mode, out_scale=1.0, aux=None, ldaux=0, naux_fwd=0,
-             nact_bwd=0, aux_scale=1.0):
+             nact_bwd=0, aux_scale=1.0, planes=0):
     a = _lib.SrGemmArgs()
     set_gemm_args(a, A, B, C, M, N, K, bias, group, act, mode, out_scale, aux, naux_fwd, nact_bwd, aux_scale, (lda, ldb, ldc, ldaux))
-    PROFILE.launch("sr_mlp_gemm_nt", a, _lib.stream_of(C), M >= 128 and N > 32, (M, N, K, mode, group))
-
-
-_TnProblem = collections.namedtuple("_TnProblem", "Z ldz A lda R N K lddw group dW db accumulate")
-
-
-def _tn_workspace(R, N, lddw):
+    a.planes = planes
+    rows = M * max(planes, 1)
+    PROFILE.launch("sr_mlp_gemm_nt", a, _lib.stream_of(C), rows >= 128 and N > 32, (rows, N, K, mode, group))
+
+
+_TnProblem = collections.namedtuple("_TnProblem", "Z ldz A lda R N K lddw group dW db accumulate planes", defaults=(0,))
+
+
+_TN_ROWS_ANY = 2 ** 31 - 1
+_TN_STEP_ROWS = 32
+
+
+def _tn_workspace(R, N, lddw, planes=0):
     splits = ctypes.c_int32(0)
-    ws = _lib.raw("sr_mlp_gemm_tn_workspace_floats")(R, N, lddw, ctypes.byref(splits))
+    query = _lib.raw("sr_mlp_gemm_tn_workspace_floats")
+    if planes:
+        query(_TN_ROWS_ANY, N, lddw, ctypes.byref(splits))
+        full = splits.value
+        if lddw <= 64:
+            query(R, N, lddw, ctypes.byref(splits))
+            per_plane = min(full, max(splits.value, math.ceil((2.0 * R) ** (1.0 / 3.0))), -(-R // _TN_STEP_ROWS))
+        else:
+            query(R * (planes + 1), N, lddw, ctypes.byref(splits))
+            per_plane = min(splits.value, -(-full // planes))
+        per_plane = max(1, per_plane)
+        return planes * per_plane * N * lddw, planes * per_plane
+    ws = query(R, N, lddw, ctypes.byref(splits))
     return max(int(ws), 1), splits.value
 
 
-def _set_tn_args(a, Z, ldz, A, lda, R, N, K, lddw, group, dW, db, accumulate, partial, ws, splits):
+def _set_tn_args(a, Z, ldz, A, lda, R, N, K, lddw, group, dW, db, accumulate, partial, ws, splits, planes=0):
     a.Z, a.ldz, a.A, a.lda, a.dW, a.lddw, a.partial = Z.data_ptr(), ldz, A.data_ptr(), lda, dW.data_ptr(), lddw, partial
     a.R, a.N, a.K, a.splits, a.accumulate = R, N, K, splits, 1 if accumulate else 0
-    a.db, a.db_partial, a.group = db.data_ptr(), partial + 4 * ws, group
-
-
-def _gemm_tn(Z, ldz, A, lda, R, N, K, lddw, group=1, dW=None, db=None, accumulate=False):
-    ws, splits = _tn_workspace(R, N, lddw)
+    a.db, a.db_partial, a.group, a.planes = _lib.ptr(db), 0 if planes else partial + 4 * ws, group, planes
+
+
+def _gemm_tn(Z, ldz, A, lda, R, N, K, lddw, group=1, dW=None, db=None, accumulate=False, planes=0):
+    ws, splits = _tn_workspace(R, N, lddw, planes)
     if dW is None:
         dW = torch.empty((N, lddw), dtype=torch.float32, device=Z.device)
-    partial = torch.empty((ws + splits * N,), dtype=torch.float32, device=Z.device)
+    partial = torch.empty((ws + (0 if planes else splits * N),), dtype=torch.float32, device=Z.device)
     if db is None:
         db = torch.empty((N,), dtype=torch.float32, device=Z.device)
     a = _lib.SrGemmTnArgs()
-    _set_tn_args(a, Z, ldz, A, lda, R, N, K, lddw, group, dW, db, accumulate, partial.data_ptr(), ws, splits)
-    PROFILE.launch("sr_mlp_gemm_tn", a, _lib.stream_of(Z), R >= 128 and N > 32, (R, N, K, "tn", group))
+    _set_tn_args(a, Z, ldz, A, lda, R, N, K, lddw, group, dW, db, accumulate, partial.data_ptr(), ws, splits, planes)
+    rows = R * max(planes, 1)
+    PROFILE.launch("sr_mlp_gemm_tn", a, _lib.stream_of(Z), rows >= 128 and N > 32, (rows, N, K, "tn", group))
     return dW, db
 
 
@@ -208,7 +227,7 @@
         total += (ws + splits * p.N + 3) // 4 * 4
     partial = torch.empty((total,), dtype=torch.float32, device=problems[0].Z.device)
     for a, p, (ws, splits, off) in zip(g.p, problems, sizes):
-        _set_tn_args(a, *p, partial.data_ptr() + 4 * off, ws, splits)
+        _set_tn_args(a, *p[:12], partial.data_ptr() + 4 * off, ws, splits)
     _lib.call("sr_mlp_gemm_tn_group", ctypes.byref(g), _lib.stream_of(partial))
 
 
@@ -237,7 +256,7 @@
             _debug_delay(device, DEBUG_TN_DELAY_MS)
         if len(problems) == 1:
             p = problems[0]
-            _gemm_tn(*p[:9], dW=p.dW, db=p.db, accumulate=p.accumulate)
+            _gemm_tn(*p[:9], dW=p.dW, db=p.db, accumulate=p.accumulate, planes=p.planes)
         else:
             _gemm_tn_group(problems)
     for p in problems:
@@ -364,6 +383,55 @@
         if grouped:
             _launch_on_tn_stream(A0.device, grouped)
     return A0bar, dWs, dbs
+
+
+TANGENT_ONLY_REVERSE = True
+_PLANE_BYTES_MAX = 1 << 32
+
+
+def tangent_only_reverse_ok(spec, A0, acts, group):
+    if not TANGENT_ONLY_REVERSE or group not in (2, 4):
+        return False
+    if any(L.act not in (ACT_RELU, ACT_NONE) or L.nfill or L.out_scale != 1.0 for L in spec.layers):
+        return False
+    P = A0.shape[0] // group
+    widest = max([A0.stride(0)] + [a.stride(0) for a in acts if a is not None] + [pad4(L.N) for L in spec.layers])
+    return P * group * widest * 4 < _PLANE_BYTES_MAX
+
+
+def reverse_tangent_planes(spec, A0, WTs, acts, Ybar, group, need_param_grad=True, Ws=None, bs=None):
+    _check_mat(Ybar, "Ybar")
+    planes = group - 1
+    R = A0.shape[0]
+    P = R // group
+    nl = len(spec.layers)
+    dWs, dbs = [None] * nl, [None] * nl
+    Zbar = Ybar
+    dev = A0.device
+    seg = _bias_segments(bs[0], R, group) if bs is not None else None
+    with _lib.on_device(dev):
+        for l in range(nl - 1, -1, -1):
+            L = spec.layers[l]
+            X = A0 if l == 0 else acts[l - 1]
+            if need_param_grad:
+                route, sink = _weight_gradient_route(l, L, Ws, bs, seg, None)
+                if sink is not None:
+                    p = _TnProblem(Zbar, Zbar.stride(0), X, X.stride(0), P, L.N, L.K, pad4(L.K), group, *sink, planes)
+                    if route == _DW_SIDE:
+                        _launch_on_tn_stream(dev, [p])
+                    else:
+                        _gemm_tn(*p[:9], dW=p.dW, db=p.db, accumulate=p.accumulate, planes=planes)
+                else:
+                    dWs[l], db = _gemm_tn(Zbar, Zbar.stride(0), X, X.stride(0), P, L.N, L.K, pad4(L.K), group, planes=planes)
+                    dbs[l] = torch.zeros((seg[0], L.N), dtype=torch.float32, device=dev) if route == _DW_SEGMENTED else db
+            if l > 0:
+                Pv = spec.layers[l - 1]
+                Znew = torch.empty((planes * P, pad4(L.K)), dtype=torch.float32, device=dev)
+                _gemm_nt(Zbar, Zbar.stride(0), WTs[l], WTs[l].stride(0), Znew, Znew.stride(0), P, L.K, L.N, None, 1, Pv.act,
+                         EPI_BWD, out_scale=Pv.out_scale, aux=acts[l - 1], ldaux=acts[l - 1].stride(0), nact_bwd=Pv.N,
+                         aux_scale=Pv.out_scale, planes=planes)
+                Zbar = Znew
+    return dWs, dbs
 
 
 def transpose_padded(W, K):
diff --git a/selfreconcode_amd/model/Deformer.py b/selfreconcode_amd/model/Deformer.py
--- a/selfreconcode_amd/model/Deformer.py
+++ b/selfreconcode_amd/model/Deformer.py
@@ -452,16 +452,23 @@
         P = flat.shape[0]
         if dbar is None and Jbar is None:
             return (None,) * (7 + 2 * nl)
+        need_par = any(ctx.needs_input_grad[7:])
+        need_x = ctx.needs_input_grad[2]
+        need_in = need_x or (ctx.needs_input_grad[3] and ctx.E > 0)
+        WTs = [me.transposed_of(Ws[l], spec.layers[l].K) for l in range(nl)]
+        acts_full = acts + [None]
+        if dbar is None and not need_in and me.tangent_only_reverse_ok(spec, A0, acts, 4):
+            if not need_par:
+                return (None,) * (7 + 2 * nl)
+            ybar = torch.zeros((3, P, 4), dtype=torch.float32, device=flat.device)
+            ybar[:, :, :3] = Jbar.permute(2, 0, 1)
+            dWs, dbs = me.reverse_tangent_planes(spec, A0, WTs, acts_full, ybar.view(3 * P, 4), 4, need_par, Ws, list(wb[nl:]))
+            return (None,) * 7 + tuple(dWs) + tuple(dbs)
         ybar = torch.zeros((P, 4, 4), dtype=torch.float32, device=flat.device)
         if dbar is not None:
             ybar[:, 0, :3] = dbar.reshape(-1, 3)
         if Jbar is not None:
             ybar[:, 1:4, :3] = Jbar.transpose(1, 2)
-        WTs = [me.transposed_of(Ws[l], spec.layers[l].K) for l in range(nl)]
-        acts_full = acts + [None]
-        need_par = any(ctx.needs_input_grad[7:])
-        need_x = ctx.needs_input_grad[2]
-        need_in = need_x or (ctx.needs_input_grad[3] and ctx.E > 0)
         A0bar, dWs, dbs = me.reverse(spec, A0, WTs, acts_full, ybar.view(P * 4, 4), 4, need_in, need_par, Ws, list(wb[nl:]))
         if not need_par:
             dWs, dbs = [None] * nl, [None] * nl
```
